# davidfang00/opticalflowdiffusion

Hardware: AMD Instinct MI355X
Metric: UNet denoise steps/sec @ 2x436x1024 flow, bs=16 (higher is better)
Workload: dtype bf16

## Files before the change

opticalflowdiffusion_amd/csrc/attn_bwd.hip:

```cpp
#include "blocks.h"

namespace ofd {

typedef __attribute__((ext_vector_type(8))) __bf16 bf16x8;
typedef __attribute__((ext_vector_type(16))) float f32x16;

__device__ __forceinline__ void a_unpack8(const uint4& v, float* f) {
    const uint32_t w[4] = {v.x, v.y, v.z, v.w};
#pragma unroll
    for (int j = 0; j < 4; ++j) {
        f[2 * j] = bf2f((bf16_t)(w[j] & 0xffffu));
        f[2 * j + 1] = bf2f((bf16_t)(w[j] >> 16));
    }
}
__device__ __forceinline__ uint4 a_pack8(const float* f) {
    return make_uint4(f2bf2(f[0], f[1]), f2bf2(f[2], f[3]), f2bf2(f[4], f[5]), f2bf2(f[6], f[7]));
}
__device__ __forceinline__ void load32(const bf16_t* p, float (&f)[32]) {
#pragma unroll
    for (int u = 0; u < 4; ++u) a_unpack8(*(const uint4*)(p + u * 8), &f[u * 8]);
}
__device__ __forceinline__ void store32(bf16_t* p, const float (&f)[32]) {
#pragma unroll
    for (int u = 0; u < 4; ++u) *(uint4*)(p + u * 8) = a_pack8(&f[u * 8]);
}

__global__ void __launch_bounds__(256) fa_bwd_delta_kernel(const bf16_t* __restrict__ o, const bf16_t* __restrict__ dout, float* __restrict__ delta, int n, size_t total) {
    for (size_t i = (size_t)blockIdx.x * 256 + threadIdx.x; i < total; i += (size_t)gridDim.x * 256) {
        const size_t pix = i >> 2;
        const int h = (int)(i & 3);
        float a[32], g[32];
        load32(o + pix * 128 + h * 32, a);
        load32(dout + pix * 128 + h * 32, g);
        float s = 0.0f;
#pragma unroll
        for (int j = 0; j < 32; ++j) s += a[j] * g[j];
        const size_t b = pix / n, q = pix % n;
        delta[(b * 4 + h) * n + q] = s;
    }
}

constexpr int FB_T = 64;
__device__ __forceinline__ int perm_slot(int idx) {
    const int kb = idx >> 5, kk = idx & 31, s = kk >> 4, a = (kk >> 3) & 1, hh = (kk >> 2) & 1, bb = kk & 3;
    return kb * 32 + s * 16 + hh * 8 + a * 4 + bb;
}
__device__ __forceinline__ void stage_transposed(unsigned char* lds, int u, int slot, const uint4& v) {
    const uint32_t w[4] = {v.x, v.y, v.z, v.w};
#pragma unroll
    for (int j = 0; j < 4; ++j) {
        *(bf16_t*)(lds + (u * 8 + 2 * j) * 144 + slot * 2) = (bf16_t)(w[j] & 0xffffu);
        *(bf16_t*)(lds + (u * 8 + 2 * j + 1) * 144 + slot * 2) = (bf16_t)(w[j] >> 16);
    }
}
__device__ __forceinline__ bf16x8 acc_to_bf16(const f32x16& a, int s) {
    bf16x8 f;
#pragma unroll
    for (int j = 0; j < 8; ++j) f[j] = (__bf16)a[8 * s + j];
    return f;
}

__global__ void __launch_bounds__(256) fa_bwd_dq_kernel(const bf16_t* __restrict__ qkv, const bf16_t* __restrict__ dout, const float* __restrict__ lse,
                                                        const float* __restrict__ delta, bf16_t* __restrict__ dqkv, int n, float scale) {
    __shared__ __attribute__((aligned(16))) unsigned char k_lds[FB_T * 80], v_lds[FB_T * 80], kt_lds[32 * 144];
    const int tid = threadIdx.x, lane = tid & 63, wave = tid >> 6, l31 = lane & 31, half = lane >> 5;
    const int bh = blockIdx.y, b = bh / 4, h = bh % 4;
    const int q0 = blockIdx.x * 128 + wave * 32;
    const bf16_t* base = qkv + (size_t)b * n * 384;
    const int qi = min(q0 + l31, n - 1);
    bf16x8 qf[2], gf[2];
#pragma unroll
    for (int s = 0; s < 2; ++s) {
        qf[s] = *(const bf16x8*)(base + (size_t)qi * 384 + h * 32 + s * 16 + half * 8);
        gf[s] = *(const bf16x8*)(dout + ((size_t)b * n + qi) * 128 + h * 32 + s * 16 + half * 8);
    }
    const float c2 = scale * 1.4426950408889634f;
    const float lse_q = lse[(size_t)bh * n + qi] * 1.4426950408889634f, dl_q = delta[(size_t)bh * n + qi] * scale;
    f32x16 dq_acc;
#pragma unroll
    for (int r = 0; r < 16; ++r) dq_acc[r] = 0.0f;
    for (int j0 = 0; j0 < n; j0 += FB_T) {
        __syncthreads();
        {
            const int key = tid >> 2, u = tid & 3;
            const int kg = min(j0 + key, n - 1);
            const uint4 kv = *(const uint4*)(base + (size_t)kg * 384 + 128 + h * 32 + u * 8);
            const uint4 vv = *(const uint4*)(base + (size_t)kg * 384 + 256 + h * 32 + u * 8);
            *(uint4*)(k_lds + key * 80 + u * 16) = kv;
            *(uint4*)(v_lds + key * 80 + u * 16) = vv;
            stage_transposed(kt_lds, u, perm_slot(key), kv);
        }
        __syncthreads();
#pragma unroll
        for (int kb = 0; kb < 2; ++kb) {
            f32x16 s_acc, p_acc;
#pragma unroll
            for (int r = 0; r < 16; ++r) { s_acc[r] = 0.0f; p_acc[r] = 0.0f; }
#pragma unroll
            for (int s = 0; s < 2; ++s) {
                const bf16x8 kf = *(const bf16x8*)(k_lds + (kb * 32 + l31) * 80 + (s * 16 + half * 8) * 2);
                const bf16x8 vf = *(const bf16x8*)(v_lds + (kb * 32 + l31) * 80 + (s * 16 + half * 8) * 2);
                s_acc = __builtin_amdgcn_mfma_f32_32x32x16_bf16(kf, qf[s], s_acc, 0, 0, 0);
                p_acc = __builtin_amdgcn_mfma_f32_32x32x16_bf16(vf, gf[s], p_acc, 0, 0, 0);
            }
#pragma unroll
            for (int r = 0; r < 16; ++r)
                s_acc[r] = __builtin_amdgcn_exp2f(__builtin_fmaf(s_acc[r], c2, -lse_q)) * __builtin_fmaf(p_acc[r], scale, -dl_q);
            if (j0 + FB_T > n) {
#pragma unroll
                for (int r = 0; r < 16; ++r)
                    if (j0 + kb * 32 + (r & 3) + 8 * (r >> 2) + 4 * half >= n) s_acc[r] = 0.0f;
            }
#pragma unroll
            for (int s = 0; s < 2; ++s) {
                const bf16x8 ktf = *(const bf16x8*)(kt_lds + l31 * 144 + (kb * 32 + s * 16 + half * 8) * 2);
                dq_acc = __builtin_amdgcn_mfma_f32_32x32x16_bf16(ktf, acc_to_bf16(s_acc, s), dq_acc, 0, 0, 0);
            }
        }
    }
    const int q = q0 + l31;
    if (q < n) {
        bf16_t* dst = dqkv + ((size_t)b * n + q) * 384 + h * 32;
#pragma unroll
        for (int g = 0; g < 4; ++g)
            *(uint2*)(dst + 8 * g + 4 * half) = make_uint2(f2bf2(dq_acc[4 * g], dq_acc[4 * g + 1]), f2bf2(dq_acc[4 * g + 2], dq_acc[4 * g + 3]));
    }
}

__global__ void __launch_bounds__(256) fa_bwd_dkv_kernel(const bf16_t* __restrict__ qkv, const bf16_t* __restrict__ dout, const float* __restrict__ lse,
                                                         const float* __restrict__ delta, bf16_t* __restrict__ dqkv, int n, float scale) {
    __shared__ __attribute__((aligned(16))) unsigned char q_lds[FB_T * 80], g_lds[FB_T * 80], qt_lds[32 * 144], gt_lds[32 * 144];
    __shared__ float lse_s[FB_T], dl_s[FB_T];
    const int tid = threadIdx.x, lane = tid & 63, wave = tid >> 6, l31 = lane & 31, half = lane >> 5;
    const int bh = blockIdx.y, b = bh / 4, h = bh % 4;
    const int k0 = blockIdx.x * 128 + wave * 32;
    const bf16_t* base = qkv + (size_t)b * n * 384;
    const int ki = min(k0 + l31, n - 1);
    bf16x8 kf[2], vf[2];
#pragma unroll
    for (int s = 0; s < 2; ++s) {
        kf[s] = *(const bf16x8*)(base + (size_t)ki * 384 + 128 + h * 32 + s * 16 + half * 8);
        vf[s] = *(const bf16x8*)(base + (size_t)ki * 384 + 256 + h * 32 + s * 16 + half * 8);
    }
    f32x16 dk_acc, dv_acc;
#pragma unroll
    for (int r = 0; r < 16; ++r) { dk_acc[r] = 0.0f; dv_acc[r] = 0.0f; }
    const float c2 = scale * 1.4426950408889634f;
    for (int i0 = 0; i0 < n; i0 += FB_T) {
        __syncthreads();
        {
            const int qq = tid >> 2, u = tid & 3;
            const bool ok = i0 + qq < n;
            const int qg = min(i0 + qq, n - 1);
            const uint4 qv = *(const uint4*)(base + (size_t)qg * 384 + h * 32 + u * 8);
            uint4 gv = *(const uint4*)(dout + ((size_t)b * n + qg) * 128 + h * 32 + u * 8);
            if (!ok) gv = make_uint4(0u, 0u, 0u, 0u);
            *(uint4*)(q_lds + qq * 80 + u * 16) = qv;
            *(uint4*)(g_lds + qq * 80 + u * 16) = gv;
            const int slot = perm_slot(qq);
            stage_transposed(qt_lds, u, slot, qv);
            stage_transposed(gt_lds, u, slot, gv);
            if (u == 0) {
                lse_s[qq] = ok ? lse[(size_t)bh * n + qg] * 1.4426950408889634f : 3.0e38f;
                dl_s[qq] = ok ? delta[(size_t)bh * n + qg] * scale : 0.0f;
            }
        }
        __syncthreads();
#pragma unroll
        for (int qb = 0; qb < 2; ++qb) {
            f32x16 s_acc, p_acc;
#pragma unroll
            for (int r = 0; r < 16; ++r) { s_acc[r] = 0.0f; p_acc[r] = 0.0f; }
#pragma unroll
            for (int s = 0; s < 2; ++s) {
                const bf16x8 qfr = *(const bf16x8*)(q_lds + (qb * 32 + l31) * 80 + (s * 16 + half * 8) * 2);
                const bf16x8 gfr = *(const bf16x8*)(g_lds + (qb * 32 + l31) * 80 + (s * 16 + half * 8) * 2);
                s_acc = __builtin_amdgcn_mfma_f32_32x32x16_bf16(qfr, kf[s], s_acc, 0, 0, 0);
                p_acc = __builtin_amdgcn_mfma_f32_32x32x16_bf16(gfr, vf[s], p_acc, 0, 0, 0);
            }
#pragma unroll
            for (int r = 0; r < 16; ++r) {
                const int qq = qb * 32 + (r & 3) + 8 * (r >> 2) + 4 * half;
                const float p = __builtin_amdgcn_exp2f(__builtin_fmaf(s_acc[r], c2, -lse_s[qq]));
                s_acc[r] = p;
                p_acc[r] = p * __builtin_fmaf(p_acc[r], scale, -dl_s[qq]);
            }
#pragma unroll
            for (int s = 0; s < 2; ++s) {
                const bf16x8 gtf = *(const bf16x8*)(gt_lds + l31 * 144 + (qb * 32 + s * 16 + half * 8) * 2);
                const bf16x8 qtf = *(const bf16x8*)(qt_lds + l31 * 144 + (qb * 32 + s * 16 + half * 8) * 2);
                dv_acc = __builtin_amdgcn_mfma_f32_32x32x16_bf16(gtf, acc_to_bf16(s_acc, s), dv_acc, 0, 0, 0);
                dk_acc = __builtin_amdgcn_mfma_f32_32x32x16_bf16(qtf, acc_to_bf16(p_acc, s), dk_acc, 0, 0, 0);
            }
        }
    }
    const int key = k0 + l31;
    if (key < n) {
        bf16_t* dst = dqkv + ((size_t)b * n + key) * 384 + h * 32;
#pragma unroll
        for (int g = 0; g < 4; ++g) {
            *(uint2*)(dst + 128 + 8 * g + 4 * half) = make_uint2(f2bf2(dk_acc[4 * g], dk_acc[4 * g + 1]), f2bf2(dk_acc[4 * g + 2], dk_acc[4 * g + 3]));
            *(uint2*)(dst + 256 + 8 * g + 4 * half) = make_uint2(f2bf2(dv_acc[4 * g], dv_acc[4 * g + 1]), f2bf2(dv_acc[4 * g + 2], dv_acc[4 * g + 3]));
        }
    }
}

int k_flash_attention_bwd(const bf16_t* qkv, const bf16_t* o, const bf16_t* dout, const float* lse, bf16_t* dqkv, float* delta, int B, int n,
                          hipStream_t s) {
    const size_t total = (size_t)B * n * 4;
    size_t gb = (total + 255) / 256;
    if (gb > 4096) gb = 4096;
    const float scale = 0.17677669529663687f;
    fa_bwd_delta_kernel<<<(int)gb, 256, 0, s>>>(o, dout, delta, n, total);
    fa_bwd_dq_kernel<<<dim3(cdiv(n, 128), B * 4), 256, 0, s>>>(qkv, dout, lse, delta, dqkv, n, scale);
    fa_bwd_dkv_kernel<<<dim3(cdiv(n, 128), B * 4), 256, 0, s>>>(qkv, dout, lse, delta, dqkv, n, scale);
    OFD_LAUNCH_CHECK();
    return OFD_OK;
}

}
using namespace ofd;

extern "C" size_t ofd_la_workspace_floats(int B, int n) { return (size_t)B * 4 * (size_t)la_fwd_parts(B, n) * 1088; }
extern "C" size_t ofd_la_bwd_workspace_floats(int B, int n) { return la_bwd_workspace_floats(B, n); }
extern "C" int ofd_linear_attention_core(const void* qkv, void* out, float* ctx, float* ml, float* workspace, int B, int n, void* stream) {
    OFD_CHECK_ARG(qkv && out && ctx && ml && workspace && B > 0 && n > 0, "linear_attention_core: bad argument");
    return k_linear_attention_core((const bf16_t*)qkv, workspace, ctx, (bf16_t*)out, B, n, (hipStream_t)stream, ml);
}
extern "C" int ofd_linear_attention_core_backward(const void* qkv, const void* dout, const float* ctx, const float* ml, void* dqkv, float* workspace,
                                                  int B, int n, void* stream) {
    OFD_CHECK_ARG(qkv && dout && ctx && ml && dqkv && workspace && B > 0 && n > 0, "linear_attention_core_backward: bad argument");
    return k_linear_attention_core_bwd((const bf16_t*)qkv, (const bf16_t*)dout, ctx, ml, (bf16_t*)dqkv, workspace, B, n, (hipStream_t)stream);
}
static inline bool al16(const void* p) { return ((uintptr_t)p & 15) == 0; }
extern "C" int ofd_la_weight_prep(const float* wqkv, const float* g, const float* wout, void* wq, void* wkv, void* woutp, int C, void* stream) {
    OFD_CHECK_ARG(wqkv && wq && wkv && (woutp == nullptr) == (wout == nullptr), "la_weight_prep: null argument (wout and woutp go together)");
    OFD_CHECK_ARG(C == 64 || C == 128, "la_weight_prep: C=%d (64 or 128)", C);
    OFD_CHECK_ARG(al16(wq) && al16(wkv) && al16(woutp), "la_weight_prep: weight buffers must be 16-byte aligned");
    return k_la_weight_prep(wqkv, g, wout, (bf16_t*)wq, (bf16_t*)wkv, (bf16_t*)woutp, C, (hipStream_t)stream);
}
extern "C" int ofd_linear_attention_block(const void* x, const void* wq, const void* wkv, const void* woutp, const float* bias, const float* g2,
                                          float* partial, void* ctxfrag, void* y, int B, int n, int C, float eps_pre, float eps_post, void* stream) {
    OFD_CHECK_ARG(x && wq && wkv && woutp && bias && g2 && partial && ctxfrag && y, "linear_attention_block: null argument");
    OFD_CHECK_ARG(C == 64 || C == 128, "linear_attention_block: C=%d (64 or 128)", C);
    OFD_CHECK_ARG(B > 0 && n > 0, "linear_attention_block: B=%d n=%d", B, n);
    OFD_CHECK_ARG(al16(x) && al16(y) && al16(wq) && al16(wkv) && al16(woutp) && al16(ctxfrag), "linear_attention_block: x, y, ctxfrag and the weights must be 16-byte aligned");
    return k_linear_attention_fused((const bf16_t*)x, (const bf16_t*)wq, (const bf16_t*)wkv, (const bf16_t*)woutp, bias, g2, partial, (bf16_t*)ctxfrag,
                                    (bf16_t*)y, B, n, C, eps_pre, eps_post, (hipStream_t)stream);
}
extern "C" int ofd_linear_attention_block_train(const void* x, const void* wq, const void* wkv, const void* woutp, const float* bias, const float* g_pre,
                                                const float* g2, float* partial, void* ctxfrag, float* ctx, float* ml, void* xn, void* qkv, void* o2,
                                                void* y, int B, int n, int C, float eps_pre, float eps_post, void* stream) {
    OFD_CHECK_ARG(x && wq && wkv && woutp && bias && g_pre && g2 && partial && ctxfrag && ctx && ml && xn && qkv && o2 && y,
                  "linear_attention_block_train: null argument");
    OFD_CHECK_ARG(C == 64, "linear_attention_block_train: C=%d (64)", C);
    OFD_CHECK_ARG(B > 0 && n > 0, "linear_attention_block_train: B=%d n=%d", B, n);
    OFD_CHECK_ARG(al16(x) && al16(y) && al16(wq) && al16(wkv) && al16(woutp) && al16(ctxfrag) && al16(xn) && al16(qkv) && al16(o2),
                  "linear_attention_block_train: x, y, xn, qkv, o2, ctxfrag and the weights must be 16-byte aligned");
    return k_linear_attention_fused_train((const bf16_t*)x, (const bf16_t*)wq, (const bf16_t*)wkv, (const bf16_t*)woutp, bias, g_pre, g2, partial,
                                          (bf16_t*)ctxfrag, ctx, ml, (bf16_t*)xn, (bf16_t*)qkv, (bf16_t*)o2, (bf16_t*)y, B, n, C, eps_pre, eps_post,
                                          (hipStream_t)stream);
}
extern "C" int ofd_linear_attention_core_proj(const void* qkv, void* out, float* ctx, float* ml, float* workspace, const void* wo, const float* bo,
                                              void* o2, int C, int B, int n, void* stream) {
    OFD_CHECK_ARG(qkv && ctx && ml && workspace && wo && o2, "linear_attention_core_proj: null argument");
    OFD_CHECK_ARG(C == 128, "linear_attention_core_proj: C=%d (128: the only width the executor runs this form at)", C);
    OFD_CHECK_ARG(B > 0 && n > 0, "linear_attention_core_proj: B=%d n=%d", B, n);
    OFD_CHECK_ARG(al16(qkv) && al16(out) && al16(wo) && al16(o2) && al16(bo), "linear_attention_core_proj: qkv, out, o2, wo and bo must be 16-byte aligned");
    return k_linear_attention_core((const bf16_t*)qkv, workspace, ctx, (bf16_t*)out, B, n, (hipStream_t)stream, ml, (const bf16_t*)wo, bo, (bf16_t*)o2, C);
}
extern "C" int ofd_linear_attention_block_backward(const void* qkv, const void* do2, const float* ctx, const float* ml, float* workspace, const void* xn,
                                                   const void* wqkv_t, float* dw_acc, void* dxn, const void* wo_fwd, const void* wo_t, float* dwo_acc,
                                                   float* dbo, const void* wq_fwd, int C, int B, int n, void* stream) {
    OFD_CHECK_ARG(qkv && do2 && ctx && ml && workspace && xn && wqkv_t && dw_acc && dxn && wo_fwd && wo_t && dwo_acc && dbo && wq_fwd,
                  "linear_attention_block_backward: null argument");
    OFD_CHECK_ARG(C == 64, "linear_attention_block_backward: C=%d (64)", C);
    OFD_CHECK_ARG(B > 0 && n > 0, "linear_attention_block_backward: B=%d n=%d", B, n);
    OFD_CHECK_ARG(al16(qkv) && al16(do2) && al16(xn) && al16(dxn) && al16(wqkv_t) && al16(wo_fwd) && al16(wo_t) && al16(wq_fwd),
                  "linear_attention_block_backward: qkv, do2, xn, dxn and the weights must be 16-byte aligned");
    return k_linear_attention_block_bwd((const bf16_t*)qkv, (const bf16_t*)do2, ctx, ml, workspace, B, n, (hipStream_t)stream, (const bf16_t*)xn,
                                        (const bf16_t*)wqkv_t, dw_acc, (bf16_t*)dxn, (const bf16_t*)wo_fwd, (const bf16_t*)wo_t, dwo_acc, dbo,
                                        (const bf16_t*)wq_fwd);
}
extern "C" int ofd_flash_attention(const void* qkv, void* out, float* lse, int B, int n, void* stream) {
    OFD_CHECK_ARG(qkv && out && B > 0 && n > 0, "flash_attention: bad argument");
    return k_flash_attention((const bf16_t*)qkv, (bf16_t*)out, B, n, (hipStream_t)stream, lse);
}
extern "C" int ofd_flash_attention_backward(const void* qkv, const void* out, const void* dout, const float* lse, void* dqkv, float* delta, int B,
                                            int n, void* stream) {
    OFD_CHECK_ARG(qkv && out && dout && lse && dqkv && delta && B > 0 && n > 0, "flash_attention_backward: bad argument");
    return k_flash_attention_bwd((const bf16_t*)qkv, (const bf16_t*)out, (const bf16_t*)dout, lse, (bf16_t*)dqkv, delta, B, n, (hipStream_t)stream);
}
```

opticalflowdiffusion_amd/csrc/blocks.h:

```cpp
#pragma once
#include "common.h"

namespace ofd {

struct MlpDesc {
    const float* weight;
    const float* bias;
    int n_out;
    int offset;
};

struct FcFuse { const float* w; const float* b; float* out; };
bool conv_fc_fuse_supported(const ofd_conv_args* a, int out_dim);
int conv_forward_impl(const ofd_conv_args* a, hipStream_t s, int pool2 = 0, const bf16_t* residual_b = nullptr, const FcFuse* fc = nullptr);
bool conv_pool2_supported(const ofd_conv_args* a);
bool conv_residual_b_supported(const ofd_conv_args* a);
int k_wt_transpose(const bf16_t* w, bf16_t* wt, int taps, int Cin, int Cout, hipStream_t s);
int k_conv_wgrad(const ofd_conv_args* a, const bf16_t* dy, float* dw, hipStream_t s, float* dbias = nullptr);
int k_conv7_wgrad(const bf16_t* x16, const bf16_t* dy, float* dw, int B, int H, int W, hipStream_t s, float* dbias = nullptr, int channels = 16);
int k_channel_sum(const bf16_t* dy, float* out, size_t npix, int C, hipStream_t s);
int k_wgrad_finish(const float* acc, const float* w_raw, float* dst, int Cout, int Cin, int Cin_pad, int ksize, float ws_eps, int unshuffle,
                   int accumulate, hipStream_t s);
int k_grad_scatter(const bf16_t* D, int Ctot, int ch_off, bf16_t* dst, int C, int B, int H, int W, int mode, int p1, int p2, int accumulate,
                   hipStream_t s);

struct ofd_weight_prep_desc {
    const float* w;
    void* out;
    int Cout, Cin, Cin_pad, ksize;
    float ws_eps;
    int unshuffle;
    int block0;
};
int k_conv_weight_prep_batched(const ofd_weight_prep_desc* d_descs, int n, int total_blocks, hipStream_t s);
int k_wt_transpose_batched(const ofd_weight_prep_desc* d_descs, int n, int total_blocks, hipStream_t s);
int k_pack_input(const float* x, int Cx, const float* cond, int Cc, bf16_t* out, int B, int H, int W, hipStream_t s, int cpad = 16, int ax = 0, int ac = 0);
int k_time_mlp(const int64_t* t, const float* w1, const float* b1, const float* w2, const float* b2, float* temb,
               float* temb_silu, int B, int dim, hipStream_t s);
int k_block_mlp(const float* temb_silu, const MlpDesc* descs, int n_desc, float* ss, int B, int tdim, int ss_stride, hipStream_t s);
int k_gn_finalize(const float* partial, int B, int H, int W, int C, const float* gamma, const float* beta, const float* ss,
                  int ss_stride, int ss_offset, float* a_out, float* s_out, hipStream_t s, float* stats_out = nullptr);
int k_resblock_out(const bf16_t* h, const float* a, const float* sft, const bf16_t* x, bf16_t* out, int B, int H, int W, int C, hipStream_t s);
int k_layernorm_c(const bf16_t* x, const float* g, const bf16_t* res, bf16_t* out, size_t npix, int C, float eps, hipStream_t s);
int la_parts(int B, int n);
int k_linear_attention_core(const bf16_t* qkv, float* partial, float* ctx, bf16_t* out, int B, int n, hipStream_t s, float* ml_out = nullptr,
                            const bf16_t* wo = nullptr, const float* bo = nullptr, bf16_t* o2 = nullptr, int C = 0);
int la_fused_blocks(int n, int B);
int la_fwd_parts(int B, int n);
int k_linear_attention_fused_train(const bf16_t* x, const bf16_t* wq, const bf16_t* wkv, const bf16_t* woutp, const float* bias, const float* g_pre,
                                   const float* g2, float* partial, bf16_t* ctxfrag, float* ctx, float* ml, bf16_t* xn, bf16_t* qkv, bf16_t* o2,
                                   bf16_t* y, int B, int n, int C, float eps_pre, float eps_post, hipStream_t s);
int k_la_weight_prep(const float* wqkv, const float* g, const float* wout, bf16_t* wq, bf16_t* wkv, bf16_t* woutp, int C, hipStream_t s);
int k_linear_attention_fused(const bf16_t* x, const bf16_t* wq, const bf16_t* wkv, const bf16_t* woutp, const float* bias, const float* g2,
                             float* partial, bf16_t* ctxfrag, bf16_t* y, int B, int n, int C, float eps_pre, float eps_post, hipStream_t s);
int k_flash_attention(const bf16_t* qkv, bf16_t* out, int B, int n, hipStream_t s, float* lse = nullptr);
int k_final_conv(const bf16_t* x, const float* w, const float* bias, float* out, int B, int H, int W, int C, int out_dim, hipStream_t s, int out_mode = 0,
                 float out_div = 1.0f);
int k_nhwc_to_nchw(const bf16_t* x, float* out, int B, int H, int W, int C, hipStream_t s);
int k_nchw_to_nhwc(const float* x, bf16_t* out, int B, int H, int W, int C, hipStream_t s);

int k_affine_silu(const bf16_t* h, const float* a, const float* s, bf16_t* out, int B, int H, int W, int C, hipStream_t st);
size_t gn_bwd_workspace_floats(int B, int H, int W, int C);
int k_gn_silu_backward(const bf16_t* g, const bf16_t* h, const float* a, const float* s, const float* stats, const float* gamma,
                       const float* beta, const float* ss, int ss_stride, int ss_offset, bf16_t* dh, float* dgamma, float* dbeta, float* dss,
                       float* workspace, int B, int H, int W, int C, hipStream_t st, float* dconv_bias = nullptr);
int k_layernorm_c_bwd(const bf16_t* x, const float* gw, const bf16_t* dy, bf16_t* dx, float* dg, size_t npix, int C, float eps, int accumulate,
                      hipStream_t st, const bf16_t* extra = nullptr);
int k_final_conv_bwd(const bf16_t* x, const float* w, const float* dy, bf16_t* dx, float* dw, float* db, int B, int H, int W, int C, int out_dim,
                     hipStream_t st, const float* bias = nullptr, int out_mode = 0, float out_div = 1.0f);
int k_conv7_dgrad(const bf16_t* dy, const bf16_t* wt, int cin_pad, float* dx, int cx, int B, int H, int W, float scale, hipStream_t s);
int k_block_mlp_bwd(const float* dss, const float* temb_silu, const float* weight, int n_out, int offset, float* dweight, float* dbias, float* dts,
                    int B, int tdim, int ss_stride, hipStream_t st);
int k_time_mlp_bwd(const int64_t* t, const float* temb, const float* dts, const float* w1, const float* b1, const float* w2, float* dw1, float* db1,
                   float* dw2, float* db2, float* scratch, int B, int dim, hipStream_t st);
int k_grad_add(bf16_t* dst, const bf16_t* src, size_t elems, int accumulate, hipStream_t st);

size_t la_bwd_workspace_floats(int B, int n);
int k_linear_attention_core_bwd(const bf16_t* qkv, const bf16_t* dout, const float* ctx, const float* ml, bf16_t* dqkv, float* workspace, int B, int n,
                                hipStream_t s);
int k_linear_attention_block_bwd(const bf16_t* qkv, const bf16_t* do2, const float* ctx, const float* ml, float* workspace, int B, int n, hipStream_t s,
                                 const bf16_t* xn, const bf16_t* wt, float* dw, bf16_t* dxn, const bf16_t* wo_fwd, const bf16_t* wo_t, float* dwo,
                                 float* dbo, const bf16_t* wq);
int k_flash_attention_bwd(const bf16_t* qkv, const bf16_t* o, const bf16_t* dout, const float* lse, bf16_t* dqkv, float* delta, int B, int n,
                          hipStream_t s);

}
```

opticalflowdiffusion_amd/csrc/la_fused.hip:

```cpp
#include <cstdlib>
#include <type_traits>
#include "blocks.h"
#include "la_common.h"

namespace ofd {

template <int C>
struct XRaw {
    u32x4 v[C / 16];
};

template <int C>
__device__ __forceinline__ void load_raw_x(const bf16_t* __restrict__ xrow, XRaw<C>& r, int half) {
#pragma unroll
    for (int s = 0; s < C / 16; ++s) r.v[s] = *(const u32x4*)(xrow + 16 * s + 8 * half);
}

typedef __bf16 la_bf16x2 __attribute__((ext_vector_type(2)));
template <int C>
__device__ __forceinline__ void norm_stats(const XRaw<C>& r, float eps, float& rstd, float& off) {
    const la_bf16x2 one = __builtin_bit_cast(la_bf16x2, 0x3f803f80u);
    float s1 = 0.0f, s2 = 0.0f;
#pragma unroll
    for (int s = 0; s < C / 16; ++s)
#pragma unroll
        for (int j = 0; j < 4; ++j) {
            const la_bf16x2 w = __builtin_bit_cast(la_bf16x2, (uint32_t)r.v[s][j]);
            s1 = __builtin_amdgcn_fdot2_f32_bf16(w, one, s1, false);
            s2 = __builtin_amdgcn_fdot2_f32_bf16(w, w, s2, false);
        }
    s1 += __shfl_xor(s1, 32, 64);
    s2 += __shfl_xor(s2, 32, 64);
    const float mean = s1 * (1.0f / C);
    const float var = fmaxf(__builtin_fmaf(-mean, mean, s2 * (1.0f / C)), 0.0f);
    rstd = rsqrtf(var + eps);
    off = -mean * rstd;
}
template <int C>
__device__ __forceinline__ void norm_x(const XRaw<C>& r, float eps, bf16x8 (&xs)[C / 16]) {
    float rstd, off;
    norm_stats<C>(r, eps, rstd, off);
#pragma unroll
    for (int s = 0; s < C / 16; ++s)
#pragma unroll
        for (int j = 0; j < 4; ++j) {
            const uint32_t w = r.v[s][j];
            xs[s][2 * j] = (__bf16)__builtin_fmaf(bf2f((bf16_t)(w & 0xffffu)), rstd, off);
            xs[s][2 * j + 1] = (__bf16)__builtin_fmaf(bf2f((bf16_t)(w >> 16)), rstd, off);
        }
}

template <int C>
__device__ __forceinline__ void norm_x_gain(const XRaw<C>& r, float eps, const float* __restrict__ g, int half, bf16x8 (&xs)[C / 16]) {
    float rstd, off;
    norm_stats<C>(r, eps, rstd, off);
#pragma unroll
    for (int s = 0; s < C / 16; ++s) {
        const float4 g0 = *(const float4*)(g + 16 * s + 8 * half), g1 = *(const float4*)(g + 16 * s + 8 * half + 4);
        const float gg[8] = {g0.x, g0.y, g0.z, g0.w, g1.x, g1.y, g1.z, g1.w};
#pragma unroll
        for (int j = 0; j < 4; ++j) {
            const uint32_t w = r.v[s][j];
            xs[s][2 * j] = (__bf16)(__builtin_fmaf(bf2f((bf16_t)(w & 0xffffu)), rstd, off) * gg[2 * j]);
            xs[s][2 * j + 1] = (__bf16)(__builtin_fmaf(bf2f((bf16_t)(w >> 16)), rstd, off) * gg[2 * j + 1]);
        }
    }
}

constexpr int LA_PART_PITCH = 64 + 32 * 36;
__device__ __forceinline__ void la_store_part(float* lds, float* __restrict__ o, float m, float l, const f32x16& ctxT, int tid, int wave, int l31,
                                              int half) {
    float* mine = lds + wave * LA_PART_PITCH;
    const float l_tot = l + __shfl_xor(l, 32, 64);
    if (half == 0) {
        mine[l31] = m;
        mine[32 + l31] = l_tot;
    }
#pragma unroll
    for (int g = 0; g < 4; ++g)
        *(float4*)(mine + 64 + l31 * 36 + 8 * g + 4 * half) = make_float4(ctxT[4 * g], ctxT[4 * g + 1], ctxT[4 * g + 2], ctxT[4 * g + 3]);
    __syncthreads();
    const int d = tid >> 3, e0 = (tid & 7) * 4;
    float mw[4], M = -3.0e38f;
#pragma unroll
    for (int w = 0; w < 4; ++w) {
        mw[w] = lds[w * LA_PART_PITCH + d];
        M = fmaxf(M, mw[w]);
    }
    float4 a = make_float4(0.0f, 0.0f, 0.0f, 0.0f);
    float ls = 0.0f;
#pragma unroll
    for (int w = 0; w < 4; ++w) {
        const float wt = __expf(mw[w] - M);
        const float4 v = *(const float4*)(lds + w * LA_PART_PITCH + 64 + d * 36 + e0);
        a.x += v.x * wt;
        a.y += v.y * wt;
        a.z += v.z * wt;
        a.w += v.w * wt;
        ls += lds[w * LA_PART_PITCH + 32 + d] * wt;
    }
    *(float4*)(o + 64 + d * 32 + e0) = a;
    if ((tid & 7) == 0) {
        o[d] = M;
        o[32 + d] = ls;
    }
    __syncthreads();
}

__device__ __forceinline__ void ctx_state_init(f32x16 (&ctxT)[4], float (&m)[4], float (&l)[4]) {
#pragma unroll
    for (int hd = 0; hd < 4; ++hd) {
        m[hd] = -3.0e38f;
        l[hd] = 0.0f;
#pragma unroll
        for (int r = 0; r < 16; ++r) ctxT[hd][r] = 0.0f;
    }
}
__device__ __forceinline__ f32x16 ctx_mask_rows(f32x16 ka, int tile, int n, int half) {
    if (tile * 32 + 32 > n) {
#pragma unroll
        for (int r = 0; r < 16; ++r)
            if (tile * 32 + acc_row(r, half) >= n) ka[r] = -3.0e38f;
    }
    return ka;
}
__device__ __forceinline__ float ctx_tile_max(const f32x16& ka) {
    float mt = -3.0e38f;
#pragma unroll
    for (int r = 0; r < 16; ++r) mt = fmaxf(mt, ka[r]);
    return fmaxf(mt, __shfl_xor(mt, 32, 64));
}
__device__ __forceinline__ void ctx_update(f32x16& ctxT, const f32x16& va, const f32x16& p) {
#pragma unroll
    for (int s2 = 0; s2 < 2; ++s2) ctxT = __builtin_amdgcn_mfma_f32_32x32x16_bf16(acc_frag(va, s2), acc_frag(p, s2), ctxT, 0, 0, 0);
}

template <int C, bool TRAIN>
__global__ void __launch_bounds__(256, 2) la_ctx_fused_kernel(const bf16_t* __restrict__ x, const bf16_t* __restrict__ wkv,
                                                           float* __restrict__ partial, int n, float eps, float defer,
                                                           const float* __restrict__ g, bf16_t* __restrict__ xn_out, bf16_t* __restrict__ qkv_out) {
    extern __shared__ __attribute__((aligned(16))) unsigned char smem[];
    constexpr int KS = C / 16;
    const int tid = threadIdx.x, lane = tid & 63, wave = tid >> 6, l31 = lane & 31, half = lane >> 5;
    for (int i = tid; i < (C / 8) * 256; i += 256) ((uint4*)smem)[i] = ((const uint4*)wkv)[i];
    float* s_g = (float*)(smem + (C / 8) * 256 * 16);
    if constexpr (TRAIN)
        for (int i = tid; i < C; i += 256) s_g[i] = g[i];
    __syncthreads();
    const int b = blockIdx.y, wave_id = blockIdx.x * 4 + wave, nw = gridDim.x * 4, ntiles = (n + 31) / 32;

    f32x16 ctxT[4];
    float m[4], l[4];
    ctx_state_init(ctxT, m, l);
    const bf16_t* xb = x + (size_t)b * n * C;
    XRaw<C> raw_next;
    load_raw_x<C>(xb + (size_t)min(wave_id * 32 + l31, n - 1) * C, raw_next, half);
    for (int tile = wave_id; tile < ntiles; tile += nw) {
        asm volatile("" ::: "memory");
        const XRaw<C> raw = raw_next;
        load_raw_x<C>(xb + (size_t)min((tile + nw) * 32 + l31, n - 1) * C, raw_next, half);
        bf16x8 xs[KS];
        const int pix = tile * 32 + l31;
        if constexpr (TRAIN) {
            norm_x_gain<C>(raw, eps, s_g, half, xs);
            if (pix < n) {
                bf16_t* xrow = xn_out + ((size_t)b * n + pix) * C;
#pragma unroll
                for (int s = 0; s < KS; ++s) *(bf16x8*)(xrow + 16 * s + 8 * half) = xs[s];
            }
        } else {
            norm_x<C>(raw, eps, xs);
        }
        if constexpr (TRAIN) {
            bf16_t* qrow = qkv_out + ((size_t)b * n + min(pix, n - 1)) * 384 + 128;
#pragma unroll
            for (int blk = 0; blk < 8; ++blk) {
                f32x16 t;
#pragma unroll
                for (int r = 0; r < 16; ++r) t[r] = 0.0f;
#pragma unroll
                for (int s = 0; s < KS; ++s)
                    t = __builtin_amdgcn_mfma_f32_32x32x16_bf16(*(const bf16x8*)(smem + ((size_t)(2 * s + half) * 256 + blk * 32 + l31) * 16), xs[s], t, 0, 0, 0);
                store_acc_rows(t, qrow + blk * 32, half, pix < n);
            }
        }
#pragma unroll
        for (int hd = 0; hd < 4; ++hd) {
            f32x16 ka, va;
#pragma unroll
            for (int r = 0; r < 16; ++r) { ka[r] = 0.0f; va[r] = 0.0f; }
#pragma unroll
            for (int s = 0; s < KS; ++s) {
                const bf16x8 wk = *(const bf16x8*)(smem + ((size_t)(2 * s + half) * 256 + hd * 32 + l31) * 16);
                const bf16x8 wv = *(const bf16x8*)(smem + ((size_t)(2 * s + half) * 256 + 128 + hd * 32 + l31) * 16);
                ka = __builtin_amdgcn_mfma_f32_32x32x16_bf16(xs[s], wk, ka, 0, 0, 0);
                va = __builtin_amdgcn_mfma_f32_32x32x16_bf16(xs[s], wv, va, 0, 0, 0);
            }
            if constexpr (TRAIN) {
#pragma unroll
                for (int r = 0; r < 16; ++r) ka[r] = bf2f(f2bf(ka[r]));
            }
            ka = ctx_mask_rows(ka, tile, n, half);
            const float mt = ctx_tile_max(ka);
            const bool move = mt > m[hd] + defer;
            if (__builtin_amdgcn_ballot_w64(move)) {
                const float m_new = move ? mt : m[hd];
                const float f = __expf(m[hd] - m_new);
                m[hd] = m_new;
                l[hd] *= f;
#pragma unroll
                for (int r = 0; r < 16; ++r) ctxT[hd][r] *= f;
            }
            float ps = 0.0f;
            const float m2 = m[hd] * LA_LOG2E;
#pragma unroll
            for (int r = 0; r < 16; ++r) {
                const float p = __builtin_amdgcn_exp2f(__builtin_fmaf(ka[r], LA_LOG2E, -m2));
                ka[r] = p;
                ps += p;
            }
            l[hd] += ps;
            ctx_update(ctxT[hd], va, ka);
            if constexpr (TRAIN) {
#pragma unroll
                for (int r = 0; r < 16; ++r) ka[r] -= (float)(__bf16)ka[r];
                ctx_update(ctxT[hd], va, ka);
            }
        }
    }
    __syncthreads();
#pragma unroll
    for (int hd = 0; hd < 4; ++hd)
        la_store_part((float*)smem, partial + ((size_t)(b * 4 + hd) * gridDim.x + blockIdx.x) * 1088, m[hd], l[hd], ctxT[hd], tid, wave, l31, half);
}

__global__ void __launch_bounds__(256, 2) la_ctx_stored_kernel(const bf16_t* __restrict__ qkv, float* __restrict__ partial, int n) {
    const int tid = threadIdx.x, lane = tid & 63, wave = tid >> 6, l31 = lane & 31, half = lane >> 5;
    const int b = blockIdx.y, wave_id = blockIdx.x * 4 + wave, nw = gridDim.x * 4, ntiles = (n + 31) / 32;
    bf16x8 ident[2];
#pragma unroll
    for (int s2 = 0; s2 < 2; ++s2)
#pragma unroll
        for (int j = 0; j < 8; ++j) ident[s2][j] = (__bf16)((16 * s2 + 8 * half + j == l31) ? 1.0f : 0.0f);
    f32x16 ctxT[4];
    float m[4], l[4];
    ctx_state_init(ctxT, m, l);
    const bf16_t* qb = qkv + (size_t)b * n * 384;
    for (int tile = wave_id; tile < ntiles; tile += nw) {
        u32x4 kr[8], vr[8];
        {
            const bf16_t* row = qb + (size_t)min(tile * 32 + l31, n - 1) * 384 + 128 + 8 * half;
#pragma unroll
            for (int i = 0; i < 8; ++i) kr[i] = *(const u32x4*)(row + 16 * i);
#pragma unroll
            for (int i = 0; i < 8; ++i) vr[i] = *(const u32x4*)(row + 128 + 16 * i);
        }
#pragma unroll
        for (int hd = 0; hd < 4; ++hd) {
            f32x16 ka, va;
#pragma unroll
            for (int r = 0; r < 16; ++r) { ka[r] = 0.0f; va[r] = 0.0f; }
#pragma unroll
            for (int s2 = 0; s2 < 2; ++s2) {
                ka = __builtin_amdgcn_mfma_f32_32x32x16_bf16(__builtin_bit_cast(bf16x8, kr[hd * 2 + s2]), ident[s2], ka, 0, 0, 0);
                va = __builtin_amdgcn_mfma_f32_32x32x16_bf16(__builtin_bit_cast(bf16x8, vr[hd * 2 + s2]), ident[s2], va, 0, 0, 0);
            }
            ka = ctx_mask_rows(ka, tile, n, half);
            const float mt = ctx_tile_max(ka);
            const float m_new = fmaxf(m[hd], mt);
            const float f = __expf(m[hd] - m_new);
            m[hd] = m_new;
            float ps = 0.0f;
            const float m2 = m_new * LA_LOG2E;
#pragma unroll
            for (int r = 0; r < 16; ++r) {
                const float p = bf2f(f2bf(__builtin_amdgcn_exp2f(__builtin_fmaf(ka[r], LA_LOG2E, -m2))));
                ka[r] = p;
                ps += p;
            }
            l[hd] = l[hd] * f + ps;
#pragma unroll
            for (int r = 0; r < 16; ++r) ctxT[hd][r] *= f;
            ctx_update(ctxT[hd], va, ka);
        }
    }
    __shared__ __attribute__((aligned(16))) float part_s[4 * LA_PART_PITCH];
#pragma unroll
    for (int hd = 0; hd < 4; ++hd)
        la_store_part(part_s, partial + ((size_t)(b * 4 + hd) * gridDim.x + blockIdx.x) * 1088, m[hd], l[hd], ctxT[hd], tid, wave, l31, half);
}

int launch_la_ctx_stored(const bf16_t* qkv, float* partial, int B, int n, hipStream_t s) {
    const int gx = la_fused_blocks(n, B);
    la_ctx_stored_kernel<<<dim3(gx, B), 256, 0, s>>>(qkv, partial, n);
    return gx;
}

constexpr int LA_MAX_PARTS = 256;
template <class Out>
__global__ void __launch_bounds__(256) la_ctx_combine_kernel(const float* __restrict__ partial, Out* __restrict__ out, int nparts, float inv_n,
                                                             float* __restrict__ ml_out) {
    constexpr bool FRAG = std::is_same<Out, bf16_t>::value;
    __shared__ float red[8][32], M[32], Linv[32], w_s[LA_MAX_PARTS][32];
    const int tid = threadIdx.x, bh = blockIdx.x, dd = tid & 31, grp = tid >> 5;
    const float* base = partial + (size_t)bh * nparts * 1088;
    float mx = -3.0e38f;
    for (int c0 = grp; c0 < nparts; c0 += 32) {
        float t[4];
#pragma unroll
        for (int k = 0; k < 4; ++k) t[k] = base[(size_t)min(c0 + 8 * k, nparts - 1) * 1088 + dd];
#pragma unroll
        for (int k = 0; k < 4; ++k) mx = fmaxf(mx, t[k]);
    }
    red[grp][dd] = mx;
    __syncthreads();
    if (tid < 32) {
        float m = red[0][tid];
#pragma unroll
        for (int g = 1; g < 8; ++g) m = fmaxf(m, red[g][tid]);
        M[tid] = m;
    }
    __syncthreads();
    const bool use_ws = nparts <= LA_MAX_PARTS;
    float l = 0.0f;
    for (int c0 = grp; c0 < nparts; c0 += 32) {
        float tm[4], tl[4];
#pragma unroll
        for (int k = 0; k < 4; ++k) {
            const size_t o = (size_t)min(c0 + 8 * k, nparts - 1) * 1088;
            tm[k] = base[o + dd];
            tl[k] = base[o + 32 + dd];
        }
#pragma unroll
        for (int k = 0; k < 4; ++k)
            if (c0 + 8 * k < nparts) {
                const float w = __expf(tm[k] - M[dd]);
                if (use_ws) w_s[c0 + 8 * k][dd] = w;
                l += tl[k] * w;
            }
    }
    __syncthreads();
    red[grp][dd] = l;
    __syncthreads();
    if (tid < 32) {
        float t = red[0][tid];
#pragma unroll
        for (int g = 1; g < 8; ++g) t += red[g][tid];
        Linv[tid] = 1.0f / t;
        if (!FRAG && ml_out && blockIdx.y == 0) {
            ml_out[(size_t)bh * 64 + tid] = M[tid];
            ml_out[(size_t)bh * 64 + 32 + tid] = 1.0f / t;
        }
    }
    __syncthreads();
    const int i = blockIdx.y * 256 + tid;
    int d, e;
    if constexpr (FRAG) {
        const int j = i & 7, lane = (i >> 3) & 63, s2 = i >> 9;
        d = 16 * s2 + 8 * (j >> 2) + 4 * (lane >> 5) + (j & 3);
        e = lane & 31;
    } else {
        d = i >> 5;
        e = i & 31;
    }
    float a = 0.0f;
    for (int c0 = 0; c0 < nparts; c0 += 8) {
        float v[8];
#pragma unroll
        for (int k = 0; k < 8; ++k) v[k] = base[(size_t)min(c0 + k, nparts - 1) * 1088 + 64 + d * 32 + e];
        if (use_ws) {
#pragma unroll
            for (int k = 0; k < 8; ++k)
                if (c0 + k < nparts) a += v[k] * w_s[c0 + k][d];
        } else {
            float mc[8];
#pragma unroll
            for (int k = 0; k < 8; ++k) mc[k] = base[(size_t)min(c0 + k, nparts - 1) * 1088 + d];
#pragma unroll
            for (int k = 0; k < 8; ++k)
                if (c0 + k < nparts) a += v[k] * __expf(mc[k] - M[d]);
        }
    }
    const float c = a * Linv[d] * inv_n;
    if constexpr (FRAG) out[(size_t)bh * 1024 + i] = f2bf(c);
    else out[(size_t)bh * 1024 + i] = c;
}
void launch_la_ctx_combine(const float* partial, float* ctx, int B, int nparts, float inv_n, float* ml_out, hipStream_t s) {
    la_ctx_combine_kernel<<<dim3(B * 4, 4), 256, 0, s>>>(partial, ctx, nparts, inv_n, ml_out);
}

template <int C, bool TRAIN>
__global__ void __launch_bounds__(256, C == 64 ? 4 : 2) la_out_fused_kernel(const bf16_t* __restrict__ x, const bf16_t* __restrict__ wq,
                                                           const bf16_t* __restrict__ woutp, const bf16_t* __restrict__ ctxfrag,
                                                           const float* __restrict__ bias, const float* __restrict__ g2,
                                                           bf16_t* __restrict__ y, int n, float eps_pre, float eps_post, float scale,
                                                           const float* __restrict__ g, bf16_t* __restrict__ o2_out) {
    extern __shared__ __attribute__((aligned(16))) unsigned char smem[];
    constexpr int KS = C / 16, RT = C / 32;
    constexpr int WQ_B = (C / 8) * 128 * 16, WO_B = 16 * C * 16, CF_B = 4 * 2 * 64 * 16;
    unsigned char* s_wq = smem;
    unsigned char* s_wo = smem + WQ_B;
    unsigned char* s_cf = s_wo + WO_B;
    float* s_bias = (float*)(s_cf + CF_B);
    float* s_g2 = s_bias + C;
    float* s_g = s_g2 + C;
    const int tid = threadIdx.x, lane = tid & 63, wave = tid >> 6, l31 = lane & 31, half = lane >> 5;
    const int b = blockIdx.y;
    if constexpr (TRAIN)
        for (int i = tid; i < C; i += 256) s_g[i] = g[i];
    for (int i = tid; i < WQ_B / 16; i += 256) ((uint4*)s_wq)[i] = ((const uint4*)wq)[i];
    for (int i = tid; i < WO_B / 16; i += 256) ((uint4*)s_wo)[i] = ((const uint4*)woutp)[i];
    for (int i = tid; i < CF_B / 16; i += 256) ((uint4*)s_cf)[i] = ((const uint4*)(ctxfrag + (size_t)b * 4096))[i];
    for (int i = tid; i < C; i += 256) { s_bias[i] = bias[i]; s_g2[i] = g2[i]; }
    __syncthreads();
    const int wave_id = blockIdx.x * 4 + wave, nw = gridDim.x * 4, ntiles = (n + 31) / 32;

    const bf16_t* xb = x + (size_t)b * n * C;
    XRaw<C> raw_next;
    load_raw_x<C>(xb + (size_t)min(wave_id * 32 + l31, n - 1) * C, raw_next, half);
    for (int tile = wave_id; tile < ntiles; tile += nw) {
        asm volatile("" ::: "memory");
        const int pix = tile * 32 + l31;
        const int pid = min(pix, n - 1);
        const bf16_t* xrow = xb + (size_t)pid * C;
        const XRaw<C> raw = raw_next;
        load_raw_x<C>(xb + (size_t)min((tile + nw) * 32 + l31, n - 1) * C, raw_next, half);
        bf16x8 xs[KS];
        if constexpr (TRAIN) norm_x_gain<C>(raw, eps_pre, s_g, half, xs);
        else norm_x<C>(raw, eps_pre, xs);
        f32x16 acc_o[RT];
#pragma unroll
        for (int rt = 0; rt < RT; ++rt)
#pragma unroll
            for (int r = 0; r < 16; ++r) acc_o[rt][r] = 0.0f;
#pragma unroll
        for (int hd = 0; hd < 4; ++hd) {
            f32x16 qa;
#pragma unroll
            for (int r = 0; r < 16; ++r) qa[r] = 0.0f;
#pragma unroll
            for (int s = 0; s < KS; ++s) {
                const bf16x8 wf = *(const bf16x8*)(s_wq + ((size_t)(2 * s + half) * 128 + hd * 32 + l31) * 16);
                qa = __builtin_amdgcn_mfma_f32_32x32x16_bf16(wf, xs[s], qa, 0, 0, 0);
            }
            if constexpr (TRAIN) {
#pragma unroll
                for (int r = 0; r < 16; ++r) qa[r] = bf2f(f2bf(qa[r]));
            }
            const float k = scale / softmax_d(qa, 32);
#pragma unroll
            for (int r = 0; r < 16; ++r) qa[r] *= k;
            f32x16 oa;
#pragma unroll
            for (int r = 0; r < 16; ++r) oa[r] = 0.0f;
#pragma unroll
            for (int s2 = 0; s2 < 2; ++s2) {
                const bf16x8 cf = *(const bf16x8*)(s_cf + ((size_t)(hd * 2 + s2) * 64 + lane) * 16);
                oa = __builtin_amdgcn_mfma_f32_32x32x16_bf16(cf, acc_frag(qa, s2), oa, 0, 0, 0);
            }
#pragma unroll
            for (int s2 = 0; s2 < 2; ++s2) {
                const bf16x8 of = acc_frag(oa, s2);
#pragma unroll
                for (int rt = 0; rt < RT; ++rt) {
                    const bf16x8 wf = *(const bf16x8*)(s_wo + ((size_t)((hd * 2 + s2) * 2 + half) * C + rt * 32 + l31) * 16);
                    acc_o[rt] = __builtin_amdgcn_mfma_f32_32x32x16_bf16(wf, of, acc_o[rt], 0, 0, 0);
                }
            }
        }
        float sum = 0.0f;
#pragma unroll
        for (int rt = 0; rt < RT; ++rt)
#pragma unroll
            for (int g = 0; g < 4; ++g) {
                const float4 bv = *(const float4*)(s_bias + rt * 32 + 8 * g + 4 * half);
                acc_o[rt][4 * g] += bv.x; acc_o[rt][4 * g + 1] += bv.y; acc_o[rt][4 * g + 2] += bv.z; acc_o[rt][4 * g + 3] += bv.w;
                if constexpr (TRAIN) {
#pragma unroll
                    for (int k = 0; k < 4; ++k) acc_o[rt][4 * g + k] = bf2f(f2bf(acc_o[rt][4 * g + k]));
                }
                sum += (acc_o[rt][4 * g] + acc_o[rt][4 * g + 1]) + (acc_o[rt][4 * g + 2] + acc_o[rt][4 * g + 3]);
            }
        if constexpr (TRAIN) {
            bf16_t* orow = o2_out + ((size_t)b * n + min(pix, n - 1)) * C;
#pragma unroll
            for (int rt = 0; rt < RT; ++rt) store_acc_rows(acc_o[rt], orow + rt * 32, half, pix < n);
        }
        sum += __shfl_xor(sum, 32, 64);
        const float mean = sum * (1.0f / C);
        float q = 0.0f;
#pragma unroll
        for (int rt = 0; rt < RT; ++rt)
#pragma unroll
            for (int r = 0; r < 16; ++r) { acc_o[rt][r] -= mean; q += acc_o[rt][r] * acc_o[rt][r]; }
        q += __shfl_xor(q, 32, 64);
        const float rstd = rsqrtf(q * (1.0f / C) + eps_post);
        {
            const bool ok = pix < n;
            bf16_t* yrow = y + ((size_t)b * n + min(pix, n - 1)) * C;
#pragma unroll
            for (int rt = 0; rt < RT; ++rt)
#pragma unroll
                for (int g = 0; g < 4; g += 2) {
                    const u32x4 xw = raw.v[rt * 2 + (g >> 1)];
                    const uint4 xv = make_uint4(xw[0], xw[1], xw[2], xw[3]);
                    const auto sx = __builtin_amdgcn_permlane32_swap(xv.x, xv.z, false, false);
                    const auto sy = __builtin_amdgcn_permlane32_swap(xv.y, xv.w, false, false);
                    const unsigned xq[2][2] = {{sx[0], sy[0]}, {sx[1], sy[1]}};
                    uint2 qo[2];
#pragma unroll
                    for (int k = 0; k < 2; ++k) {
                        const int c0 = rt * 32 + 8 * (g + k) + 4 * half;
                        const float4 gv = *(const float4*)(s_g2 + c0);
                        const float o0 = acc_o[rt][4 * (g + k)] * rstd * gv.x + bf2f((bf16_t)(xq[k][0] & 0xffffu));
                        const float o1 = acc_o[rt][4 * (g + k) + 1] * rstd * gv.y + bf2f((bf16_t)(xq[k][0] >> 16));
                        const float o2 = acc_o[rt][4 * (g + k) + 2] * rstd * gv.z + bf2f((bf16_t)(xq[k][1] & 0xffffu));
                        const float o3 = acc_o[rt][4 * (g + k) + 3] * rstd * gv.w + bf2f((bf16_t)(xq[k][1] >> 16));
                        qo[k] = pack_quad(o0, o1, o2, o3);
                    }
                    store_quad_pair(yrow + rt * 32 + 8 * g, qo[0], qo[1], half, ok);
                }
        }
    }
}

__global__ void __launch_bounds__(256) la_weight_prep_kernel(const float* __restrict__ wqkv, const float* __restrict__ g, const float* __restrict__ wout,
                                                             bf16_t* __restrict__ wq, bf16_t* __restrict__ wkv, bf16_t* __restrict__ woutp, int C) {
    const int total = 512 * C;
    for (int i = blockIdx.x * blockDim.x + threadIdx.x; i < total; i += gridDim.x * blockDim.x) {
        if (i < 128 * C) {
            const int j = i & 7, o = (i >> 3) & 127, c8 = i >> 10, c = c8 * 8 + j;
            wq[i] = f2bf(wqkv[(size_t)o * C + c] * (g ? g[c] : 1.0f));
        } else if (i < 384 * C) {
            const int k = i - 128 * C;
            const int j = k & 7, o = (k >> 3) & 255, c8 = k >> 11, c = c8 * 8 + j;
            wkv[k] = f2bf(wqkv[(size_t)(128 + o) * C + c] * (g ? g[c] : 1.0f));
        } else if (woutp) {
            const int k = i - 384 * C;
            const int j = k & 7, c = (k >> 3) % C, rest = (k >> 3) / C;
            const int hh = rest & 1, s2 = (rest >> 1) & 1, hd = rest >> 2;
            woutp[k] = f2bf(wout[(size_t)c * 128 + hd * 32 + 16 * s2 + 8 * (j >> 2) + 4 * hh + (j & 3)]);
        }
    }
}

constexpr float LA_DEFER = 5.545177f;
constexpr int LA_GX2_CAP = 128;
static int la_out_blocks(int n, int B) {
    int gx2 = cdiv(cdiv(n, 32), 4 * 4);
    if (gx2 < 1) gx2 = 1;
    const int cap2 = (LA_GX2_CAP * B < 1024) ? 1024 / B : LA_GX2_CAP;
    if (gx2 > cap2) gx2 = cap2;
    return gx2;
}

template <int C>
static int launch_la(const bf16_t* x, const bf16_t* wq, const bf16_t* wkv, const bf16_t* woutp, const float* bias, const float* g2,
                     float* partial, bf16_t* ctxfrag, bf16_t* y, int B, int n, float eps_pre, float eps_post, hipStream_t s) {
    constexpr int LDS1 = (C / 8) * 256 * 16;
    constexpr int LDS2 = (C / 8) * 128 * 16 + 16 * C * 16 + 4 * 2 * 64 * 16 + 2 * C * 4;
    static bool attr = false;
    if (!attr) {
        OFD_HIP(hipFuncSetAttribute((const void*)la_ctx_fused_kernel<C, false>, hipFuncAttributeMaxDynamicSharedMemorySize, LDS1));
        OFD_HIP(hipFuncSetAttribute((const void*)la_out_fused_kernel<C, false>, hipFuncAttributeMaxDynamicSharedMemorySize, LDS2));
        attr = true;
    }
    const int gx = la_fused_blocks(n, B);
    la_ctx_fused_kernel<C, false><<<dim3(gx, B), 256, LDS1, s>>>(x, wkv, partial, n, eps_pre, LA_DEFER, nullptr, nullptr, nullptr);
    la_ctx_combine_kernel<<<dim3(B * 4, 4), 256, 0, s>>>(partial, ctxfrag, gx, 1.0f / (float)n, nullptr);
    la_out_fused_kernel<C, false><<<dim3(la_out_blocks(n, B), B), 256, LDS2, s>>>(x, wq, woutp, ctxfrag, bias, g2, y, n, eps_pre, eps_post, LA_SCALE, nullptr, nullptr);
    OFD_LAUNCH_CHECK();
    return OFD_OK;
}

int k_linear_attention_fused_train(const bf16_t* x, const bf16_t* wq, const bf16_t* wkv, const bf16_t* woutp, const float* bias, const float* g_pre,
                                   const float* g2, float* partial, bf16_t* ctxfrag, float* ctx, float* ml, bf16_t* xn, bf16_t* qkv, bf16_t* o2,
                                   bf16_t* y, int B, int n, int C, float eps_pre, float eps_post, hipStream_t s) {
    if (C != 64) { set_error("linear_attention_fused_train: C=%d unsupported", C); return OFD_ERR_ARG; }
    constexpr int LDS1 = (64 / 8) * 256 * 16 + 64 * 4;
    constexpr int LDS2 = (64 / 8) * 128 * 16 + 16 * 64 * 16 + 4 * 2 * 64 * 16 + 3 * 64 * 4;
    static bool attr = false;
    if (!attr) {
        OFD_HIP(hipFuncSetAttribute((const void*)la_ctx_fused_kernel<64, true>, hipFuncAttributeMaxDynamicSharedMemorySize, LDS1));
        OFD_HIP(hipFuncSetAttribute((const void*)la_out_fused_kernel<64, true>, hipFuncAttributeMaxDynamicSharedMemorySize, LDS2));
        attr = true;
    }
    const int gx = la_fused_blocks(n, B);
    la_ctx_fused_kernel<64, true><<<dim3(gx, B), 256, LDS1, s>>>(x, wkv, partial, n, eps_pre, LA_DEFER, g_pre, xn, qkv);
    la_ctx_combine_kernel<<<dim3(B * 4, 4), 256, 0, s>>>(partial, ctxfrag, gx, 1.0f / (float)n, nullptr);
    launch_la_ctx_combine(partial, ctx, B, gx, 1.0f / (float)n, ml, s);
    la_out_fused_kernel<64, true><<<dim3(la_out_blocks(n, B), B), 256, LDS2, s>>>(x, wq, woutp, ctxfrag, bias, g2, y, n, eps_pre, eps_post, LA_SCALE, g_pre, o2);
    OFD_LAUNCH_CHECK();
    return OFD_OK;
}

int la_fused_blocks(int n, int B) {
    constexpr int total = 256;
    int gx = cdiv(cdiv(n, 32), 8);
    int cap = total / (B < 1 ? 1 : B);
    if (cap < 64) cap = 64;
    if (gx < 1) gx = 1;
    if (gx > cap) gx = cap;
    return gx;
}

int k_la_weight_prep(const float* wqkv, const float* g, const float* wout, bf16_t* wq, bf16_t* wkv, bf16_t* woutp, int C, hipStream_t s) {
    la_weight_prep_kernel<<<cdiv((woutp ? 512 : 384) * C, 256), 256, 0, s>>>(wqkv, g, wout, wq, wkv, woutp, C);
    OFD_LAUNCH_CHECK();
    return OFD_OK;
}

int k_linear_attention_fused(const bf16_t* x, const bf16_t* wq, const bf16_t* wkv, const bf16_t* woutp, const float* bias, const float* g2,
                             float* partial, bf16_t* ctxfrag, bf16_t* y, int B, int n, int C, float eps_pre, float eps_post, hipStream_t s) {
    if (C == 64) return launch_la<64>(x, wq, wkv, woutp, bias, g2, partial, ctxfrag, y, B, n, eps_pre, eps_post, s);
    if (C == 128) return launch_la<128>(x, wq, wkv, woutp, bias, g2, partial, ctxfrag, y, B, n, eps_pre, eps_post, s);
    set_error("linear_attention_fused: C=%d unsupported", C);
    return OFD_ERR_ARG;
}

}
```

opticalflowdiffusion_amd/csrc/unet.hip:

```cpp
#include <cstdlib>
#include "unet_exec.h"

using namespace ofd;

namespace ofd {

float site_eps(const ofd_unet* u, const std::string& site) {
    if (u->cfg.eps_mode == 0) return 1e-5f;
    auto ends = [&](const char* s) { std::string t(s); return site.size() >= t.size() && site.compare(site.size() - t.size(), t.size(), t) == 0; };
    if (ends(".fn.fn.to_out.1")) return 1e-3f;
    if (ends(".0.block1.proj") && site.rfind("downs.", 0) == 0) return 1e-3f;
    if (site == "mid_block1.block1.proj" || site == "final_res_block.block1.proj") return 1e-3f;
    return 1e-5f;
}

static void add_param(ofd_unet* u, const std::string& name, std::vector<int> shape) {
    size_t numel = 1;
    for (int d : shape) numel *= (size_t)d;
    Param p{name, (int)shape.size(), {1, 1, 1, 1}, numel, u->n_param_floats, false};
    for (size_t i = 0; i < shape.size(); ++i) p.shape[i] = shape[i];
    u->pindex[name] = (int)u->params.size();
    u->params.push_back(p);
    u->n_param_floats += (numel + 3) / 4 * 4;
}

static void add_conv(ofd_unet* u, const std::string& prefix, int co, int ci, int k, bool bias, float ws_eps, int unshuffle = 0) {
    add_param(u, prefix + ".weight", {co, ci, k, k});
    if (bias) add_param(u, prefix + ".bias", {co});
    ConvDesc c{prefix + ".weight", co, ci, (k == 7) ? (ci + 15) / 16 * 16 : ci, k, ws_eps, unshuffle, u->n_wbuf};
    u->n_wbuf += (size_t)k * k * c.Cin_pad * co;
    if (k == 7 && ci <= 8) {
        c.pack8_off = (long)u->n_wbuf;
        u->n_wbuf += ofd_conv_weight_elems(co, 8, 7);
    }
    u->cindex[prefix] = (int)u->convs.size();
    u->convs.push_back(c);
}

static void add_resblock(ofd_unet* u, const std::string& name, int ci, int co) {
    const int tdim = u->cfg.dim * 4;
    if (!u->cfg.no_time) {
        add_param(u, name + ".mlp.1.weight", {co * 2, tdim});
        add_param(u, name + ".mlp.1.bias", {co * 2});
    }
    add_conv(u, name + ".block1.proj", co, ci, 3, true, site_eps(u, name + ".block1.proj"));
    add_param(u, name + ".block1.norm.weight", {co});
    add_param(u, name + ".block1.norm.bias", {co});
    add_conv(u, name + ".block2.proj", co, co, 3, true, site_eps(u, name + ".block2.proj"));
    add_param(u, name + ".block2.norm.weight", {co});
    add_param(u, name + ".block2.norm.bias", {co});
    if (ci != co) add_conv(u, name + ".res_conv", co, ci, 1, true, -1.0f);
    u->ss_offset[name] = u->ss_stride;
    u->ss_stride += 2 * co;
}

static void add_linattn(ofd_unet* u, const std::string& name, int c) {
    add_conv(u, name + ".fn.fn.to_qkv", 384, c, 1, false, -1.0f);
    add_conv(u, name + ".fn.fn.to_out.0", c, 128, 1, true, -1.0f);
    add_param(u, name + ".fn.fn.to_out.1.g", {1, c, 1, 1});
    add_param(u, name + ".fn.norm.g", {1, c, 1, 1});
    if (c <= 128) {
        u->la_fused[name] = {u->n_labuf, c};
        u->n_labuf += (size_t)512 * c;
        if (c == 64) u->n_labuf += (size_t)384 * c;
    }
}

static void build_registry(ofd_unet* u) {
    const int dim = u->cfg.dim, L = u->L;
    u->dims = {dim, dim, dim * 2, dim * 4};
    if (L == 4) u->dims.push_back(dim * 8);
    const int tdim = dim * 4;
    add_conv(u, "init_conv", dim, u->cfg.channels, 7, true, -1.0f);
    u->cin_pad = u->convs.back().Cin_pad;
    if (!u->cfg.no_time) {
        add_param(u, "time_mlp.1.weight", {tdim, dim});
        add_param(u, "time_mlp.1.bias", {tdim});
        add_param(u, "time_mlp.3.weight", {tdim, tdim});
        add_param(u, "time_mlp.3.bias", {tdim});
    }
    for (int i = 0; i < L; ++i) {
        const int ci = u->dims[i], co = u->dims[i + 1];
        const std::string p = "downs." + std::to_string(i);
        add_resblock(u, p + ".0", ci, ci);
        add_resblock(u, p + ".1", ci, ci);
        add_linattn(u, p + ".2", ci);
        if (i < L - 1) add_conv(u, p + ".3.1", co, ci * 4, 1, true, -1.0f, 1);
        else add_conv(u, p + ".3", co, ci, 3, true, -1.0f);
    }
    for (int i = 0; i < L; ++i) {
        const int ci = u->dims[L - 1 - i], co = u->dims[L - i];
        const std::string p = "ups." + std::to_string(i);
        add_resblock(u, p + ".0", co + ci, co);
        add_resblock(u, p + ".1", co + ci, co);
        add_linattn(u, p + ".2", co);
        if (i < L - 1) {
            add_conv(u, p + ".3.1", ci, co, 3, true, -1.0f);
            ConvDesc& d = u->convs.back();
            d.phase_off = (long)u->n_wbuf;
            u->n_wbuf += (size_t)16 * co * ci;
        }
        else add_conv(u, p + ".3", ci, co, 3, true, -1.0f);
    }
    const int mid = u->dims[L];
    add_resblock(u, "mid_block1", mid, mid);
    add_conv(u, "mid_attn.fn.fn.to_qkv", 384, mid, 1, false, -1.0f);
    add_conv(u, "mid_attn.fn.fn.to_out", mid, 128, 1, true, -1.0f);
    add_param(u, "mid_attn.fn.norm.g", {1, mid, 1, 1});
    add_resblock(u, "mid_block2", mid, mid);
    add_resblock(u, "final_res_block", dim * 2, dim);
    add_param(u, "final_conv.weight", {u->cfg.out_dim, dim, 1, 1});
    add_param(u, "final_conv.bias", {u->cfg.out_dim});
    for (auto& kv : u->ss_offset) u->resblocks.push_back(kv.first);
}

void conv(Ctx& c, const std::string& prefix, const std::vector<SrcSpec>& srcs, Tensor out, const float* in_scale,
                 const float* in_shift, const bf16_t* residual, const bf16_t* res_act, const float* res_scale,
                 const float* res_shift, float* gn_partial, const FcFuse* fc) {
    if (c.rc != OFD_OK) return;
    const ConvDesc& d = c.u->convs[c.u->cindex.at(prefix)];
    ofd_conv_args a{};
    a.B = c.B; a.H = out.H; a.W = out.W; a.ksize = d.ksize; a.n_src = (int)srcs.size(); a.Cout = d.Cout;
    int cin = 0;
    for (size_t i = 0; i < srcs.size(); ++i) {
        a.src[i].src = srcs[i].t.p;
        a.src[i].channels = srcs[i].t.C;
        a.src[i].src_channels = srcs[i].t.C;
        a.src[i].ch_offset = 0;
        a.src[i].upsample = srcs[i].upsample;
        a.src[i].unshuffle = srcs[i].unshuffle;
        a.src[i].p1 = srcs[i].p1;
        a.src[i].p2 = srcs[i].p2;
        cin += srcs[i].t.C;
    }
    const bool pack8 = d.ksize == 7 && cin == 8 && d.pack8_off >= 0;
    if (cin != d.Cin_pad && !pack8) { set_error("conv %s: got %d input channels, expected %d", prefix.c_str(), cin, d.Cin_pad); c.rc = OFD_ERR_ARG; return; }
    a.weight = c.u->d_wbuf + (pack8 ? (size_t)d.pack8_off : d.w_off);
    a.bias = c.u->P(prefix + ".bias");
    a.in_scale = in_scale; a.in_shift = in_shift; a.residual = residual; a.res_act = res_act;
    a.res_scale = res_scale; a.res_shift = res_shift; a.out = out.p; a.gn_partial = gn_partial;
    const double px = (double)c.B * out.H * out.W;
    const double flops = 2.0 * px * d.Cout * (double)d.Cin * d.ksize * d.ksize;
    const double bytes = px * 2.0 * (d.Cout + (double)cin / ((srcs[0].upsample) ? 4 : 1)) + (double)d.ksize * d.ksize * d.Cin_pad * d.Cout * 2.0;
    const bool pp = d.ksize == 3 && d.Cout == 64 && cin == 64 && srcs.size() == 1 && !srcs[0].upsample && !residual && !res_act;
    const int cls3 = pp ? PC_CONV3_PP : (d.Cout % 128 == 0 ? PC_CONV3 : PC_CONV3_64);
    c.begin(d.ksize == 3 ? cls3 : (d.ksize == 1 ? PC_CONV1 : PC_CONV7), flops, bytes,
            prefix + " " + std::to_string(d.Cin) + "->" + std::to_string(d.Cout) + " @" + std::to_string(out.H) + "x" + std::to_string(out.W));
    RUN(conv_forward_impl(&a, c.s, 0, nullptr, fc));
    c.end();
}

static Tensor resblock(Ctx& c, const std::string& name, const std::vector<Tensor>& in, int Cout, bool keep_out = true, const FcFuse* fc = nullptr) {
    ofd_unet* u = c.u;
    const int H = in[0].H, W = in[0].W, B = c.B;
    std::vector<SrcSpec> srcs;
    int cin = 0;
    for (auto& t : in) { SrcSpec s; s.t = t; srcs.push_back(s); cin += t.C; }
    Tensor h1 = c.tmp(Cout, H, W), h2 = c.tmp(Cout, H, W);
    const size_t np = ofd_conv_gn_partial_count(B, H, W, Cout);
    float* p1 = c.tmpf(np);
    float* p2 = c.tmpf(np);
    float* a1 = c.train ? c.keepf((size_t)B * Cout) : c.tmpf((size_t)B * Cout);
    float* s1 = c.train ? c.keepf((size_t)B * Cout) : c.tmpf((size_t)B * Cout);
    float* a2 = c.train ? c.keepf((size_t)B * Cout) : c.tmpf((size_t)B * Cout);
    float* s2 = c.train ? c.keepf((size_t)B * Cout) : c.tmpf((size_t)B * Cout);
    float* st1 = c.train ? c.keepf((size_t)B * 16) : nullptr;
    float* st2 = c.train ? c.keepf((size_t)B * 16) : nullptr;
    Tensor out = keep_out ? c.keep(Cout, H, W) : c.tmp(Cout, H, W);
    if (c.rc != OFD_OK) return out;
    conv(c, name + ".block1.proj", srcs, h1, nullptr, nullptr, nullptr, nullptr, nullptr, nullptr, p1);
    c.begin(PC_GN, 0, (double)np * 4);
    RUN(k_gn_finalize(p1, B, H, W, Cout, u->P(name + ".block1.norm.weight"), u->P(name + ".block1.norm.bias"), c.ss, u->ss_stride,
                      u->ss_offset.at(name), a1, s1, c.s, st1));
    c.end();
    SrcSpec hs; hs.t = h1;
    constexpr int act1_min = 256;
    constexpr int act1_train_min = 128;
    const int amin = c.train ? act1_train_min : act1_min;
    Tensor act1;
    if (Cout >= amin) {
        act1 = c.tmp(Cout, H, W);
        if (c.rc != OFD_OK) return out;
        c.begin(PC_MISC, 0, (double)B * H * W * Cout * 4.0);
        RUN(k_affine_silu(h1.p, a1, s1, act1.p, B, H, W, Cout, c.s));
        c.end();
        hs.t = act1;
        conv(c, name + ".block2.proj", {hs}, h2, nullptr, nullptr, nullptr, nullptr, nullptr, nullptr, p2);
    } else
    conv(c, name + ".block2.proj", {hs}, h2, a1, s1, nullptr, nullptr, nullptr, nullptr, p2);
    c.begin(PC_GN, 0, (double)np * 4);
    RUN(k_gn_finalize(p2, B, H, W, Cout, u->P(name + ".block2.norm.weight"), u->P(name + ".block2.norm.bias"), nullptr, 0, 0, a2, s2, c.s, st2));
    c.end();
    if (cin != Cout) {
        conv(c, name + ".res_conv", srcs, out, nullptr, nullptr, nullptr, h2.p, a2, s2, nullptr, fc);
    } else {
        c.begin(PC_RESOUT, 0, (double)B * H * W * Cout * 6.0);
        RUN(k_resblock_out(h2.p, a2, s2, in[0].p, out.p, B, H, W, Cout, c.s));
        c.end();
    }
    if (c.train) {
        TapeRec r;
        r.kind = TK_RES; r.name = name; r.srcs = srcs; r.out = out; r.h1 = h1; r.h2 = h2;
        r.a1 = a1; r.s1 = s1; r.a2 = a2; r.s2 = s2; r.st1 = st1; r.st2 = st2; r.act1 = act1;
        u->tape.push_back(r);
    }
    return out;
}

static Tensor linattn(Ctx& c, const std::string& name, Tensor x) {
    ofd_unet* u = c.u;
    const int H = x.H, W = x.W, B = c.B, C = x.C, n = H * W;
    const size_t npix = (size_t)B * n;
    auto fit = u->la_fused.find(name);
    if (fit != u->la_fused.end() && !c.train) {
        const int nparts = la_fused_blocks(n, B);
        float* partial = c.tmpf((size_t)B * 4 * nparts * 1088);
        bf16_t* ctxfrag = (bf16_t*)c.tmpf((size_t)B * 2048);
        Tensor y = c.keep(C, H, W);
        if (c.rc != OFD_OK) return y;
        const bf16_t* base = u->d_labuf + fit->second.first;
        c.begin(PC_LINATTN, npix * 2.0 * (C * 384.0 + 2 * 4 * 32 * 32 + 128.0 * C), (double)npix * C * 2 * 3,
                name + " fused C=" + std::to_string(C) + " @" + std::to_string(H) + "x" + std::to_string(W));
        RUN(k_linear_attention_fused(x.p, base, base + (size_t)128 * C, base + (size_t)384 * C, u->P(name + ".fn.fn.to_out.0.bias"),
                                     u->P(name + ".fn.fn.to_out.1.g"), partial, ctxfrag, y.p, B, n, C, site_eps(u, name + ".fn.norm"),
                                     site_eps(u, name + ".fn.fn.to_out.1"), c.s));
        c.end();
        return y;
    }
    Tensor xn = c.tmp(C, H, W), qkv = c.tmp(384, H, W), ao = c.tmp(128, H, W), o2 = c.tmp(C, H, W);
    const int nparts = la_fwd_parts(B, n);
    if (c.train && fit != u->la_fused.end() && la_train_fused(C)) {
        float* partial = c.tmpf((size_t)B * 4 * nparts * 1088);
        bf16_t* ctxfrag = (bf16_t*)c.tmpf((size_t)B * 2048);
        float* ctx = c.keepf((size_t)B * 4 * 1024);
        float* ml = c.keepf((size_t)B * 4 * 64);
        Tensor y = c.keep(C, H, W);
        if (c.rc != OFD_OK) return y;
        const bf16_t* base = u->d_labuf + fit->second.first;
        c.begin(PC_LINATTN, npix * 2.0 * (C * 640.0 + 2 * 4 * 32 * 32 + 128.0 * C), (double)npix * C * 2 * (2 + 1 + 4 + 2),
                name + " fused (training) C=" + std::to_string(C) + " @" + std::to_string(H) + "x" + std::to_string(W));
        RUN(k_linear_attention_fused_train(x.p, base + (size_t)512 * C, base + (size_t)640 * C, base + (size_t)384 * C, u->P(name + ".fn.fn.to_out.0.bias"),
                                           u->P(name + ".fn.norm.g"), u->P(name + ".fn.fn.to_out.1.g"), partial, ctxfrag, ctx, ml, xn.p, qkv.p, o2.p, y.p,
                                           B, n, C, site_eps(u, name + ".fn.norm"), site_eps(u, name + ".fn.fn.to_out.1"), c.s));
        c.end();
        TapeRec r;
        r.kind = TK_LINATTN; r.name = name; r.x = x; r.xn = xn; r.qkv = qkv; r.ao = ao; r.o2 = o2; r.out = y; r.ctx = ctx; r.ml = ml;
        u->tape.push_back(r);
        return y;
    }
    float* partial = c.tmpf((size_t)B * 4 * nparts * 1088);
    float* ctx = c.train ? c.keepf((size_t)B * 4 * 1024) : c.tmpf((size_t)B * 4 * 1024);
    float* ml = c.train ? c.keepf((size_t)B * 4 * 64) : nullptr;
    Tensor y = c.keep(C, H, W);
    if (c.rc != OFD_OK) return y;
    c.begin(PC_LN, 0, (double)npix * C * 4);
    RUN(k_layernorm_c(x.p, u->P(name + ".fn.norm.g"), nullptr, xn.p, npix, C, site_eps(u, name + ".fn.norm"), c.s));
    c.end();
    SrcSpec s; s.t = xn;
    conv(c, name + ".fn.fn.to_qkv", {s}, qkv, nullptr, nullptr, nullptr, nullptr, nullptr, nullptr, nullptr);
    c.begin(PC_LINATTN, 4.0 * npix * 4 * 32 * 32, (double)npix * (384 + 128 + 128) * 2);
    if (C == 128) {
        const ConvDesc& d = u->convs[u->cindex.at(name + ".fn.fn.to_out.0")];
        RUN(k_linear_attention_core(qkv.p, partial, ctx, ao.p, B, n, c.s, ml, u->d_wbuf + d.w_off, u->P(name + ".fn.fn.to_out.0.bias"), o2.p, C));
        c.end();
    } else {
        RUN(k_linear_attention_core(qkv.p, partial, ctx, ao.p, B, n, c.s, ml));
        c.end();
        SrcSpec s2; s2.t = ao;
        conv(c, name + ".fn.fn.to_out.0", {s2}, o2, nullptr, nullptr, nullptr, nullptr, nullptr, nullptr, nullptr);
    }
    c.begin(PC_LN, 0, (double)npix * C * 6);
    RUN(k_layernorm_c(o2.p, u->P(name + ".fn.fn.to_out.1.g"), x.p, y.p, npix, C, site_eps(u, name + ".fn.fn.to_out.1"), c.s));
    c.end();
    if (c.train) {
        TapeRec r;
        r.kind = TK_LINATTN; r.name = name; r.x = x; r.xn = xn; r.qkv = qkv; r.ao = ao; r.o2 = o2; r.out = y; r.ctx = ctx; r.ml = ml;
        u->tape.push_back(r);
    }
    return y;
}

static Tensor midattn(Ctx& c, Tensor x) {
    ofd_unet* u = c.u;
    const int H = x.H, W = x.W, B = c.B, C = x.C, n = H * W;
    Tensor xn = c.tmp(C, H, W), qkv = c.tmp(384, H, W), ao = c.tmp(128, H, W);
    float* lse = c.train ? c.keepf((size_t)B * 4 * n) : nullptr;
    Tensor y = c.keep(C, H, W);
    if (c.rc != OFD_OK) return y;
    const size_t npix = (size_t)B * n;
    c.begin(PC_LN, 0, (double)npix * C * 4);
    RUN(k_layernorm_c(x.p, u->P("mid_attn.fn.norm.g"), nullptr, xn.p, npix, C, site_eps(u, "mid_attn.fn.norm"), c.s));
    c.end();
    SrcSpec s; s.t = xn;
    conv(c, "mid_attn.fn.fn.to_qkv", {s}, qkv, nullptr, nullptr, nullptr, nullptr, nullptr, nullptr, nullptr);
    c.begin(PC_FLASH, 4.0 * B * 4.0 * (double)n * n * 32, (double)npix * (384 + 128) * 2);
    RUN(k_flash_attention(qkv.p, ao.p, B, n, c.s, lse));
    c.end();
    SrcSpec s2; s2.t = ao;
    conv(c, "mid_attn.fn.fn.to_out", {s2}, y, nullptr, nullptr, x.p, nullptr, nullptr, nullptr, nullptr);
    if (c.train) {
        TapeRec r;
        r.kind = TK_MIDATTN; r.name = "mid_attn"; r.x = x; r.xn = xn; r.qkv = qkv; r.ao = ao; r.out = y; r.lse = lse;
        u->tape.push_back(r);
    }
    return y;
}

static void plain_conv(Ctx& c, const std::string& prefix, const std::vector<SrcSpec>& srcs, Tensor out) {
    conv(c, prefix, srcs, out, nullptr, nullptr, nullptr, nullptr, nullptr, nullptr, nullptr);
    if (c.train) {
        TapeRec r;
        r.kind = TK_CONV; r.name = prefix; r.srcs = srcs; r.out = out;
        c.u->tape.push_back(r);
    }
}

static void upsample_conv(Ctx& c, const std::string& prefix, const SrcSpec& src_up, Tensor out) {
    ofd_unet* u = c.u;
    const ConvDesc& d = u->convs[u->cindex.at(prefix)];
    if (d.phase_off < 0) { plain_conv(c, prefix, {src_up}, out); return; }
    if (c.rc != OFD_OK) return;
    const Tensor& lo = src_up.t;
    const double px = (double)c.B * out.H * out.W;
    c.begin(PC_CONVUP, 2.0 * px * d.Cout * (double)d.Cin * 9 , px * 2.0 * (d.Cout + d.Cin / 4.0),
            prefix + " " + std::to_string(d.Cin) + "->" + std::to_string(d.Cout) + " @" + std::to_string(out.H) + "x" + std::to_string(out.W) + " (4 phases)");
    {
        ofd_conv_args a{};
        a.B = c.B; a.H = lo.H; a.W = lo.W; a.ksize = 2; a.n_src = 1; a.Cout = d.Cout;
        a.src[0].src = lo.p; a.src[0].channels = lo.C; a.src[0].src_channels = lo.C;
        a.weight = u->d_wbuf + d.phase_off;
        a.bias = u->P(prefix + ".bias");
        a.out = out.p;
        a.up2_phase = 5;
        RUN(conv_forward_impl(&a, c.s));
    }
    c.end();
    if (c.train) {
        TapeRec r;
        r.kind = TK_CONV; r.name = prefix; r.srcs = {src_up}; r.out = out;
        u->tape.push_back(r);
    }
}

int run_forward(Ctx& c, const float* x, int Cx, const float* cond, int Cc, const int64_t* t, float* out, int H, int W, float* temb,
                float* temb_silu) {
    ofd_unet* u = c.u;
    const int B = c.B, dim = u->cfg.dim;
    u->taps.clear();
    u->last_B = B;
    if (c.train) u->tape.clear();
    const bool pack8 = u->convs[u->cindex.at("init_conv")].pack8_off >= 0;
    const int cpad = pack8 ? 8 : u->cin_pad;
    const int L = u->L;
    Tensor xin = c.keep(cpad, H, W);
    c.begin(PC_MISC, 0, 0);
    RUN(k_pack_input(x, Cx, cond, cond ? Cc : 0, xin.p, B, H, W, c.s, cpad, u->glue_x, u->glue_cond));
    if (!u->cfg.no_time) {
        RUN(k_time_mlp(t, u->P("time_mlp.1.weight"), u->P("time_mlp.1.bias"), u->P("time_mlp.3.weight"), u->P("time_mlp.3.bias"), temb, temb_silu, B, dim, c.s));
        RUN(k_block_mlp(temb_silu, u->d_mlp, (int)u->resblocks.size(), c.ss, B, dim * 4, u->ss_stride, c.s));
    } else {
        c.ss = nullptr;
    }
    c.end();
    Tensor r = c.keep(dim, H, W);
    { SrcSpec s; s.t = xin; plain_conv(c, "init_conv", {s}, r); }
    u->taps["init_conv"] = r;

    Tensor xcur = r;
    std::vector<Tensor> hs;
    for (int i = 0; i < L; ++i) {
        const std::string p = "downs." + std::to_string(i);
        c.reset_scratch();
        xcur = resblock(c, p + ".0", {xcur}, u->dims[i]);
        hs.push_back(xcur);
        u->taps[p + ".0"] = xcur;
        c.reset_scratch();
        Tensor x1 = resblock(c, p + ".1", {xcur}, u->dims[i]);
        u->taps[p + ".1"] = x1;
        c.reset_scratch();
        xcur = linattn(c, p + ".2", x1);
        hs.push_back(xcur);
        u->taps[p + ".2"] = xcur;
        if (i < L - 1) {
            Tensor d = c.keep(u->dims[i + 1], xcur.H / 2, xcur.W / 2);
            std::vector<SrcSpec> srcs;
            for (int sub = 0; sub < 4; ++sub) { SrcSpec s; s.t = xcur; s.unshuffle = 1; s.p1 = sub >> 1; s.p2 = sub & 1; srcs.push_back(s); }
            plain_conv(c, p + ".3.1", srcs, d);
            xcur = d;
        } else {
            Tensor d = c.keep(u->dims[i + 1], xcur.H, xcur.W);
            SrcSpec s; s.t = xcur;
            plain_conv(c, p + ".3", {s}, d);
            xcur = d;
        }
        u->taps[p + ".3"] = xcur;
    }
    c.reset_scratch();
    xcur = resblock(c, "mid_block1", {xcur}, u->dims[L]);
    u->taps["mid_block1"] = xcur;
    c.reset_scratch();
    xcur = midattn(c, xcur);
    u->taps["mid_attn"] = xcur;
    c.reset_scratch();
    xcur = resblock(c, "mid_block2", {xcur}, u->dims[L]);
    u->taps["mid_block2"] = xcur;
    for (int i = 0; i < L; ++i) {
        const std::string p = "ups." + std::to_string(i);
        const int co = u->dims[L - i], ci = u->dims[L - 1 - i];
        c.reset_scratch();
        Tensor h = hs.back(); hs.pop_back();
        xcur = resblock(c, p + ".0", {xcur, h}, co);
        u->taps[p + ".0"] = xcur;
        c.reset_scratch();
        h = hs.back(); hs.pop_back();
        xcur = resblock(c, p + ".1", {xcur, h}, co);
        u->taps[p + ".1"] = xcur;
        c.reset_scratch();
        xcur = linattn(c, p + ".2", xcur);
        u->taps[p + ".2"] = xcur;
        if (i < L - 1) {
            Tensor d = c.keep(ci, xcur.H * 2, xcur.W * 2);
            SrcSpec s; s.t = xcur; s.upsample = 1;
            upsample_conv(c, p + ".3.1", s, d);
            xcur = d;
        } else {
            Tensor d = c.keep(ci, xcur.H, xcur.W);
            SrcSpec s; s.t = xcur;
            plain_conv(c, p + ".3", {s}, d);
            xcur = d;
        }
        u->taps[p + ".3"] = xcur;
    }
    c.reset_scratch();
    const int glue = u->glue_out;
    const bool fuse_fc = !c.train && !u->debug_taps && !glue && u->cfg.out_dim == 2 && dim == 64 && ((long)H * W) % 128 == 0;
    if (fuse_fc) {
        const FcFuse fc{u->P("final_conv.weight"), u->P("final_conv.bias"), out};
        if (c.rc == OFD_OK && !c.dry) {
            if (hipMemsetAsync(out, 0, (size_t)B * 2 * H * W * sizeof(float), c.s) != hipSuccess) { set_error("unet_forward: hipMemsetAsync failed"); c.rc = OFD_ERR_HIP; }
            c.chain_ok = false;
        }
        xcur = resblock(c, "final_res_block", {xcur, r}, dim, true, &fc);
    } else {
        xcur = resblock(c, "final_res_block", {xcur, r}, dim);
        u->taps["final_res_block"] = xcur;
        c.begin(PC_MISC, 2.0 * B * H * W * dim * u->cfg.out_dim, (double)B * H * W * (dim * 2 + u->cfg.out_dim * 4));
        RUN(k_final_conv(xcur.p, u->P("final_conv.weight"), u->P("final_conv.bias"), out, B, H, W, dim, u->cfg.out_dim, c.s, glue, u->glue_div));
        c.end();
    }
    if (c.train) {
        u->ts.B = B; u->ts.H = H; u->ts.W = W; u->ts.t = t; u->ts.ss = c.ss; u->ts.temb = temb; u->ts.temb_silu = temb_silu;
        u->ts.xin = xin; u->ts.r = r; u->ts.xf = xcur; u->ts.persist_used = c.persist_used;
    }
    return c.rc;
}

size_t persist_bytes(const ofd_unet* u, int B, int H, int W) {
    auto T = [&](int C, int h, int w) { return ((size_t)B * h * w * C * 2 + 255) / 256 * 256; };
    const int L = u->L;
    size_t n = T(u->cin_pad, H, W) + T(u->dims[0], H, W);
    int h = H, w = W;
    for (int i = 0; i < L; ++i) {
        n += 3 * T(u->dims[i], h, w);
        if (i < L - 1) { h /= 2; w /= 2; }
        n += T(u->dims[i + 1], h, w);
    }
    n += 3 * T(u->dims[L], h, w);
    for (int i = 0; i < L; ++i) {
        const int co = u->dims[L - i], ci = u->dims[L - 1 - i];
        n += 3 * T(co, h, w);
        if (i < L - 1) { h *= 2; w *= 2; }
        n += T(ci, h, w);
    }
    n += T(u->dims[0], H, W);
    return n + 4096;
}

size_t scratch_bytes(const ofd_unet* u, int B, int H, int W) {
    const size_t px = (size_t)B * H * W;
    const int C = u->dims[0];
    size_t act = px * 2 * (size_t)(3 * C + C + 384 + 128 + C);
    size_t small = 4 * ofd_conv_gn_partial_count(B, H, W, u->dims[u->L]) * 4 + (size_t)B * 4 * ((size_t)(la_fwd_parts(B, H * W) > 256 ? la_fwd_parts(B, H * W) : 256) * 1088 + 1024) * 4 +
                   16 * (size_t)B * u->dims[u->L] * 4 + 64 * 1024;
    return act + small + 64 * 256;
}

size_t small_bytes(const ofd_unet* u, int B) {
    return ((size_t)B * u->ss_stride + 2 * (size_t)B * u->cfg.dim * 4) * 4 + 4096;
}

}

static void drop_graphs(ofd_unet* u);

static void upload_mlp_descs(ofd_unet* u) {
    if (u->cfg.no_time) return;
    std::vector<MlpDesc> descs;
    for (auto& name : u->resblocks) {
        MlpDesc d;
        d.weight = u->P(name + ".mlp.1.weight");
        d.bias = u->P(name + ".mlp.1.bias");
        d.n_out = (int)u->params[u->pindex.at(name + ".mlp.1.bias")].numel;
        d.offset = u->ss_offset.at(name);
        descs.push_back(d);
    }
    if (hipMemcpy(u->d_mlp, descs.data(), descs.size() * sizeof(MlpDesc), hipMemcpyHostToDevice) != hipSuccess)
        set_error("unet: uploading the time-projection descriptors failed");
}

extern "C" int ofd_unet_bind_param_buffer(ofd_unet* u, float* dev_params, size_t floats) {
    OFD_CHECK_ARG(u && dev_params, "unet_bind_param_buffer: null argument");
    OFD_CHECK_ARG(floats >= u->n_param_floats, "unet_bind_param_buffer: %zu floats, need %zu", floats, u->n_param_floats);
    OFD_CHECK_ARG(((uintptr_t)dev_params & 15) == 0, "unet_bind_param_buffer: buffer must be 16-byte aligned");
    if (u->owns_params && u->d_params) (void)hipFree(u->d_params);
    drop_graphs(u);
    if (u->d_prep) { (void)hipFree(u->d_prep); u->d_prep = nullptr; u->n_prep = 0; u->prep_blocks = 0; }
    u->d_params = dev_params;
    u->owns_params = false;
    for (auto& p : u->params) p.set = true;
    upload_mlp_descs(u);
    u->prepared = false;
    u->wt_prepared = false;
    return OFD_OK;
}

extern "C" int ofd_unet_create(const ofd_unet_config* cfg, ofd_unet** out) {
    OFD_CHECK_ARG(cfg && out, "unet_create: null argument");
    OFD_CHECK_ARG(cfg->dim == 64, "unet_create: dim=%d unsupported (the FlowDiffuser UNet is Unet(64), flow_diffuser.py:106)", cfg->dim);
    OFD_CHECK_ARG(cfg->channels >= 1 && cfg->channels <= 48, "unet_create: channels=%d (1..48)", cfg->channels);
    OFD_CHECK_ARG(cfg->out_dim >= 1 && cfg->out_dim <= 16, "unet_create: out_dim=%d (1..16)", cfg->out_dim);
    OFD_CHECK_ARG(cfg->n_levels == 0 || cfg->n_levels == 3 || cfg->n_levels == 4, "unet_create: n_levels=%d (0 or 4: dim_mults (1,2,4,8); 3: (1,2,4))",
                  cfg->n_levels);
    OFD_CHECK_ARG(cfg->n_levels != 3 || cfg->no_time == 1, "unet_create: the three-level UNet (the Autoencoder's) takes no time input (no_time=1)");
    OFD_CHECK_ARG(cfg->eps_mode == 0 || cfg->eps_mode == 1, "unet_create: eps_mode=%d", cfg->eps_mode);
    OFD_CHECK_ARG(cfg->no_time == 0 || cfg->no_time == 1, "unet_create: no_time=%d", cfg->no_time);
    ofd_unet* u = new ofd_unet();
    u->cfg = *cfg;
    u->L = cfg->n_levels == 3 ? 3 : 4;
    u->deterministic = env_int("OFD_DETERMINISTIC", 0) != 0;
    build_registry(u);
    if (hipMalloc(&u->d_params, u->n_param_floats * sizeof(float)) != hipSuccess ||
        hipMalloc(&u->d_wbuf, u->n_wbuf * sizeof(bf16_t)) != hipSuccess ||
        hipMalloc(&u->d_mlp, u->resblocks.size() * sizeof(MlpDesc)) != hipSuccess ||
        hipMalloc(&u->d_labuf, (u->n_labuf + 8) * sizeof(bf16_t)) != hipSuccess) {
        set_error("unet_create: hipMalloc failed");
        ofd_unet_destroy(u);
        return OFD_ERR_HIP;
    }
    if (hipMemset(u->d_params, 0, u->n_param_floats * sizeof(float)) != hipSuccess) {
        set_error("unet_create: hipMemset failed");
        ofd_unet_destroy(u);
        return OFD_ERR_HIP;
    }
    upload_mlp_descs(u);
    *out = u;
    return OFD_OK;
}

extern "C" void ofd_unet_destroy(ofd_unet* u) {
    if (!u) return;
    if (u->d_params && u->owns_params) (void)hipFree(u->d_params);
    if (u->d_wbuf) (void)hipFree(u->d_wbuf);
    if (u->d_mlp) (void)hipFree(u->d_mlp);
    if (u->d_labuf) (void)hipFree(u->d_labuf);
    if (u->d_wtbuf) (void)hipFree(u->d_wtbuf);
    if (u->d_wacc) (void)hipFree(u->d_wacc);
    if (u->d_fx) (void)hipFree(u->d_fx);
    if (u->d_det_miss) (void)hipFree(u->d_det_miss);
    if (u->d_prep) (void)hipFree(u->d_prep);
    if (u->d_tr) (void)hipFree(u->d_tr);
    drop_graphs(u);
    if (u->s2) {
        (void)hipStreamDestroy(u->s2);
        (void)hipEventDestroy(u->ev_fork); (void)hipEventDestroy(u->ev_join); (void)hipEventDestroy(u->ev_phase);
    }
    for (auto e : u->pool) (void)hipEventDestroy(e);
    delete u;
}

extern "C" int ofd_unet_num_params(const ofd_unet* u) { return u ? (int)u->params.size() : 0; }
extern "C" const char* ofd_unet_param_name(const ofd_unet* u, int i) {
    return (u && i >= 0 && i < (int)u->params.size()) ? u->params[i].name.c_str() : "";
}
extern "C" size_t ofd_unet_param_numel(const ofd_unet* u, int i) {
    return (u && i >= 0 && i < (int)u->params.size()) ? u->params[i].numel : 0;
}

extern "C" int ofd_unet_param_shape(const ofd_unet* u, int i, int* dims4) {
    if (!u || i < 0 || i >= (int)u->params.size() || !dims4) return 0;
    for (int k = 0; k < 4; ++k) dims4[k] = u->params[i].shape[k];
    return u->params[i].ndim;
}

extern "C" int ofd_unet_set_param(ofd_unet* u, int i, const float* dev_src, size_t numel, void* stream) {
    OFD_CHECK_ARG(u && dev_src && i >= 0 && i < (int)u->params.size(), "unet_set_param: bad argument");
    Param& p = u->params[i];
    OFD_CHECK_ARG(numel == p.numel, "unet_set_param: %s has %zu elements, got %zu", p.name.c_str(), p.numel, numel);
    OFD_HIP(hipMemcpyAsync(u->d_params + p.offset, dev_src, numel * sizeof(float), hipMemcpyDeviceToDevice, (hipStream_t)stream));
    p.set = true;
    u->prepared = false;
    u->wt_prepared = false;
    return OFD_OK;
}

extern "C" int ofd_unet_prepare(ofd_unet* u, void* stream) {
    OFD_CHECK_ARG(u, "unet_prepare: null handle");
    for (auto& p : u->params)
        if (!p.set) {
            set_error("unet_prepare: parameter %s was never set", p.name.c_str());
            return OFD_ERR_STATE;
        }
    if (!u->d_prep) {
        std::vector<ofd_weight_prep_desc> h;
        int blocks = 0;
        auto add = [&](const ConvDesc& c, size_t off, int cin_pad, int unshuffle) {
            ofd_weight_prep_desc d{u->P(c.wname), u->d_wbuf + off, c.Cout, c.Cin, cin_pad, c.ksize, c.ws_eps, unshuffle, blocks};
            h.push_back(d);
            blocks += c.Cout;
        };
        for (auto& c : u->convs) {
            add(c, c.w_off, c.Cin_pad, c.unshuffle);
            if (c.pack8_off >= 0) add(c, (size_t)c.pack8_off, 8, 0);
        }
        OFD_HIP(hipMalloc(&u->d_prep, h.size() * sizeof(ofd_weight_prep_desc)));
        OFD_HIP(hipMemcpy(u->d_prep, h.data(), h.size() * sizeof(ofd_weight_prep_desc), hipMemcpyHostToDevice));
        u->n_prep = (int)h.size();
        u->prep_blocks = blocks;
    }
    {
        int rc = k_conv_weight_prep_batched(u->d_prep, u->n_prep, u->prep_blocks, (hipStream_t)stream);
        if (rc != OFD_OK) return rc;
    }
    for (auto& c : u->convs) {
        if (c.phase_off >= 0) {
            int rc = ofd_conv_upsample_phase_weight_prep(u->P(c.wname), u->d_wbuf + c.phase_off, c.Cout, c.Cin, stream);
            if (rc != OFD_OK) return rc;
        }
    }
    for (auto& kv : u->la_fused) {
        const std::string& name = kv.first;
        const int C = kv.second.second;
        bf16_t* base = u->d_labuf + kv.second.first;
        int rc = k_la_weight_prep(u->P(name + ".fn.fn.to_qkv.weight"), u->P(name + ".fn.norm.g"), u->P(name + ".fn.fn.to_out.0.weight"),
                                  base, base + (size_t)128 * C, base + (size_t)384 * C, C, (hipStream_t)stream);
        if (rc != OFD_OK) return rc;
        if (C == 64) {
            rc = k_la_weight_prep(u->P(name + ".fn.fn.to_qkv.weight"), nullptr, nullptr, base + (size_t)512 * C, base + (size_t)640 * C, nullptr, C, (hipStream_t)stream);
            if (rc != OFD_OK) return rc;
        }
    }
    u->prepared = true;
    u->wt_prepared = false;
    return OFD_OK;
}

static size_t staging_bytes(const ofd_unet* u, int B, int H, int W) {
    auto al = [](size_t n) { return (n + 255) / 256 * 256; };
    return al((size_t)B * u->cfg.channels * H * W * 4) + al((size_t)B * 8) + al((size_t)B * u->cfg.out_dim * H * W * 4);
}

static size_t workspace_bytes_one(const ofd_unet* u, int B, int H, int W) {
    return persist_bytes(u, B, H, W) + scratch_bytes(u, B, H, W) + small_bytes(u, B) + 1024 + staging_bytes(u, B, H, W);
}

static size_t half_workspace_bytes(const ofd_unet* u, int B, int H, int W) { return (workspace_bytes_one(u, B / 2, H, W) + 255) / 256 * 256; }

extern "C" size_t ofd_unet_workspace_bytes(const ofd_unet* u, int B, int H, int W) {
    if (!u || B <= 0 || H <= 0 || W <= 0) return 0;
    const size_t one = workspace_bytes_one(u, B, H, W);
    if (B >= 2 && B % 2 == 0) { const size_t two = 2 * half_workspace_bytes(u, B, H, W); return two > one ? two : one; }
    return one;
}

static void drop_graphs(ofd_unet* u) {
    for (auto& g : u->graphs) {
        if (g.state == 2) { (void)hipGraphExecDestroy(g.exec); (void)hipGraphDestroy(g.graph); }
    }
    u->graphs.clear();
    if (u->cap_stream) { (void)hipStreamDestroy(u->cap_stream); u->cap_stream = nullptr; }
}

extern "C" int ofd_unet_set_graph(ofd_unet* u, int enabled) {
    OFD_CHECK_ARG(u, "unet_set_graph: null handle");
    u->graph_enabled = enabled != 0;
    if (!u->graph_enabled) drop_graphs(u);
    return OFD_OK;
}

extern "C" int ofd_unet_forward(ofd_unet* u, const float* x, int Cx, const float* cond, int Cc, const int64_t* t, float* out,
                                int B, int H, int W, void* workspace, size_t workspace_bytes, void* stream) {
    OFD_CHECK_ARG(u && x && (t || u->cfg.no_time) && out && workspace, "unet_forward: null argument");
    const int mult = 1 << (u->L - 1);
    OFD_CHECK_ARG(B > 0 && H > 0 && W > 0 && H % mult == 0 && W % mult == 0, "unet_forward: H=%d W=%d must be positive multiples of %d (%d 2x down-samplings, DD:95-99)",
                  H, W, mult, u->L - 1);
    OFD_CHECK_ARG(Cx + (cond ? Cc : 0) == u->cfg.channels, "unet_forward: %d + %d input channels, UNet has %d", Cx, cond ? Cc : 0, u->cfg.channels);
    if (!u->prepared) { set_error("unet_forward: call ofd_unet_prepare after setting parameters"); return OFD_ERR_STATE; }
    OFD_CHECK_WORKSPACE(workspace_bytes, ofd_unet_workspace_bytes(u, B, H, W), "unet_forward");
    OFD_CHECK_ARG(((uintptr_t)workspace & 255) == 0, "unet_forward: workspace must be 256-byte aligned");
    auto layout = [&](Ctx& c, int b, char* w_, size_t bytes, hipStream_t s_, float*& temb_, float*& temb_silu_) {
        c.u = u; c.s = s_; c.B = b;
        const size_t sb = (small_bytes(u, b) + 255) / 256 * 256;
        float* fsmall = (float*)w_;
        c.ss = fsmall;
        temb_ = fsmall + (size_t)b * u->ss_stride;
        temb_silu_ = temb_ + (size_t)b * u->cfg.dim * 4;
        c.persist = w_ + sb;
        c.persist_cap = persist_bytes(u, b, H, W);
        c.scratch = c.persist + (c.persist_cap + 255) / 256 * 256;
        c.scratch_cap = bytes - staging_bytes(u, b, H, W) - (size_t)(c.scratch - w_);
    };
    char* w = (char*)workspace;
    const bool split_auto = u->split_streams < 0 && (long)B * H * W >= (1L << 21);
    if ((u->split_streams > 0 || split_auto) && B >= 2 && B % 2 == 0 && !u->profiling && !u->graph_enabled) {
        if (!u->s2) {
            OFD_HIP(hipStreamCreateWithFlags(&u->s2, hipStreamNonBlocking));
            OFD_HIP(hipEventCreateWithFlags(&u->ev_fork, hipEventDisableTiming));
            OFD_HIP(hipEventCreateWithFlags(&u->ev_join, hipEventDisableTiming));
            OFD_HIP(hipEventCreateWithFlags(&u->ev_phase, hipEventDisableTiming));
        }
        const int hb = B / 2;
        const size_t hbytes = half_workspace_bytes(u, B, H, W);
        hipStream_t s1 = (hipStream_t)stream;
        Ctx c0, c1;
        float *te0, *ts0, *te1, *ts1;
        layout(c0, hb, w, hbytes, s1, te0, ts0);
        layout(c1, hb, w + hbytes, hbytes, u->s2, te1, ts1);
        const size_t plane = (size_t)H * W;
        c0.signal_at = u->split_offset; c0.signal_ev = u->ev_phase;
        OFD_HIP(hipEventRecord(u->ev_fork, s1));
        OFD_HIP(hipStreamWaitEvent(u->s2, u->ev_fork, 0));
        int rc = run_forward(c0, x, Cx, cond, Cc, t, out, H, W, te0, ts0), rc1 = OFD_OK;
        hipError_t he = hipSuccess;
        if (rc == OFD_OK) {
            if (!c0.signalled) he = hipEventRecord(u->ev_phase, s1);
            u->taps_half0 = u->taps;
            if (he == hipSuccess) he = hipStreamWaitEvent(u->s2, u->ev_phase, 0);
            if (he == hipSuccess)
                rc1 = run_forward(c1, x + (size_t)hb * Cx * plane, Cx, cond ? cond + (size_t)hb * Cc * plane : nullptr, Cc, t ? t + hb : nullptr,
                                  out + (size_t)hb * u->cfg.out_dim * plane, H, W, te1, ts1);
        }
        hipError_t hj = hipEventRecord(u->ev_join, u->s2);
        if (hj == hipSuccess) hj = hipStreamWaitEvent(s1, u->ev_join, 0);
        if (hj != hipSuccess) (void)hipStreamSynchronize(u->s2);
        if (he != hipSuccess || hj != hipSuccess) {
            set_error("unet_forward (split streams): %s", hipGetErrorString(he != hipSuccess ? he : hj));
            if (rc == OFD_OK && rc1 == OFD_OK) rc = OFD_ERR_HIP;
        }
        u->last_split = true;
        return rc != OFD_OK ? rc : rc1;
    }
    u->last_split = false;
    Ctx c;
    float *temb, *temb_silu;
    layout(c, B, w, workspace_bytes, (hipStream_t)stream, temb, temb_silu);
    const size_t stg = staging_bytes(u, B, H, W);
    if (!u->graph_enabled || u->profiling) return run_forward(c, x, Cx, cond, Cc, t, out, H, W, temb, temb_silu);

    auto al = [](size_t n) { return (n + 255) / 256 * 256; };
    char* sbase = w + workspace_bytes - stg;
    sbase = (char*)(((uintptr_t)sbase) & ~(uintptr_t)255);
    const size_t plane = (size_t)H * W * 4;
    float* sx = (float*)sbase;
    float* sc = sx + (size_t)B * Cx * H * W;
    int64_t* st = (int64_t*)(sbase + al((size_t)B * u->cfg.channels * plane));
    float* sout = (float*)((char*)st + al((size_t)B * 8));
    hipStream_t s_ = (hipStream_t)stream;
    OFD_HIP(hipMemcpyAsync(sx, x, (size_t)B * Cx * plane, hipMemcpyDeviceToDevice, s_));
    if (cond) OFD_HIP(hipMemcpyAsync(sc, cond, (size_t)B * Cc * plane, hipMemcpyDeviceToDevice, s_));
    if (t) OFD_HIP(hipMemcpyAsync(st, t, (size_t)B * 8, hipMemcpyDeviceToDevice, s_));
    ofd_unet::GraphEntry* e = nullptr;
    for (auto& g : u->graphs)
        if (g.workspace == workspace && g.B == B && g.H == H && g.W == W && g.Cx == Cx && g.Cc == (cond ? Cc : 0) && g.stream == s_) e = &g;
    int rc = OFD_OK;
    if (!e) {
        if (u->graphs.size() >= 8) drop_graphs(u);
        u->graphs.push_back({workspace, B, H, W, Cx, cond ? Cc : 0, s_, 0, nullptr, nullptr});
        rc = run_forward(c, sx, Cx, cond ? sc : nullptr, Cc, st, sout, H, W, temb, temb_silu);
    } else {
        if (e->state == 0) {
            if (!u->cap_stream) OFD_HIP(hipStreamCreateWithFlags(&u->cap_stream, hipStreamNonBlocking));
            OFD_HIP(hipStreamBeginCapture(u->cap_stream, hipStreamCaptureModeThreadLocal));
            c.s = u->cap_stream;
            rc = run_forward(c, sx, Cx, cond ? sc : nullptr, Cc, st, sout, H, W, temb, temb_silu);
            hipGraph_t g = nullptr;
            const hipError_t er = hipStreamEndCapture(u->cap_stream, &g);
            if (rc != OFD_OK || er != hipSuccess || !g) {
                if (g) (void)hipGraphDestroy(g);
                if (rc == OFD_OK) { set_error("unet_forward: stream capture failed: %s", hipGetErrorString(er)); rc = OFD_ERR_HIP; }
                return rc;
            }
            hipGraphExec_t ex = nullptr;
            OFD_HIP(hipGraphInstantiate(&ex, g, nullptr, nullptr, 0));
            e->graph = g; e->exec = ex; e->state = 2;
        }
        OFD_HIP(hipGraphLaunch(e->exec, s_));
    }
    if (rc != OFD_OK) return rc;
    OFD_HIP(hipMemcpyAsync(out, sout, (size_t)B * u->cfg.out_dim * plane, hipMemcpyDeviceToDevice, s_));
    return OFD_OK;
}

extern "C" int ofd_unet_set_split_streams(ofd_unet* u, int enabled, int offset_blocks) {
    OFD_CHECK_ARG(u, "unet_set_split_streams: null handle");
    u->split_streams = enabled < 0 ? -1 : (enabled != 0);
    if (offset_blocks >= 0) u->split_offset = offset_blocks;
    return OFD_OK;
}

extern "C" int ofd_unet_set_debug_taps(ofd_unet* u, int enabled) {
    OFD_CHECK_ARG(u, "unet_set_debug_taps: null handle");
    u->debug_taps = enabled != 0;
    return OFD_OK;
}

extern "C" int ofd_unet_set_glue(ofd_unet* u, int x_affine, int cond_affine, int out_mode, float out_div) {
    OFD_CHECK_ARG(u, "unet_set_glue: null handle");
    OFD_CHECK_ARG((x_affine == 0 || x_affine == 1) && (cond_affine == 0 || cond_affine == 1), "unet_set_glue: affine flags are 0 or 1");
    OFD_CHECK_ARG(out_mode >= 0 && out_mode <= 2, "unet_set_glue: out_mode=%d (0..2)", out_mode);
    OFD_CHECK_ARG(out_div > 0.0f, "unet_set_glue: out_div=%g must be positive", (double)out_div);
    u->glue_x = x_affine; u->glue_cond = cond_affine; u->glue_out = out_mode; u->glue_div = out_div;
    drop_graphs(u);
    return OFD_OK;
}

extern "C" int ofd_unet_read_tap(ofd_unet* u, const char* name, float* dst, size_t numel, void* stream) {
    OFD_CHECK_ARG(u && name && dst, "unet_read_tap: null argument");
    auto it = u->taps.find(name);
    OFD_CHECK_ARG(it != u->taps.end(), "unet_read_tap: no tap named '%s' in the last forward%s", name,
                  std::string(name) == "final_res_block" ? " (that tensor is only materialised after ofd_unet_set_debug_taps(u, 1): the final 1x1 conv normally rides on its producer)" : "");
    const Tensor& t = it->second;
    const int halves = u->last_split ? 2 : 1;
    OFD_CHECK_ARG(numel == (size_t)halves * u->last_B * t.C * t.H * t.W, "unet_read_tap: %s has %zu elements, got %zu", name,
                  (size_t)halves * u->last_B * t.C * t.H * t.W, numel);
    if (u->last_split) {
        const Tensor& t0 = u->taps_half0.at(name);
        int rc = k_nhwc_to_nchw(t0.p, dst, u->last_B, t.H, t.W, t.C, (hipStream_t)stream);
        if (rc != OFD_OK) return rc;
        dst += (size_t)u->last_B * t.C * t.H * t.W;
    }
    return k_nhwc_to_nchw(t.p, dst, u->last_B, t.H, t.W, t.C, (hipStream_t)stream);
}

extern "C" int ofd_unet_set_profiling(ofd_unet* u, int enabled) {
    OFD_CHECK_ARG(u, "unet_set_profiling: null handle");
    u->profiling = enabled != 0;
    return OFD_OK;
}
extern "C" int ofd_unet_prof_dump_path(ofd_unet* u, const char* path) {
    OFD_CHECK_ARG(u, "unet_prof_dump_path: null handle");
    u->dump_path = path ? path : "";
    return OFD_OK;
}
namespace ofd {
const char* prof_class_name(int cls) {
    static std::string names[PC_COUNT];
    static bool built = false;
    if (!built) {
        const std::string c64 = env_int("OFD_CONV_PC", 1) ? "conv3x3_pc_kernel" : "conv3x3_wp_kernel<2,2>";
        names[PC_CONV3] = "conv3x3_wp16_kernel [3x3, Cout a multiple of 128]";
        names[PC_CONV3_64] = c64 + " [3x3, Cin > 64 -> 64]";
        names[PC_CONV3_PP] = c64 + " [3x3, 64 -> 64]";
        names[PC_CONV1] = "conv1x1_wp_kernel | conv_igemm_kernel<1,BN> [1x1]";
        names[PC_CONV7] = std::string(env_int("OFD_CONV7_PERSIST", 1) ? "conv7x7_c8_persist_kernel" : "conv_igemm_kernel<8,64>") + " [7x7 init conv]";
        names[PC_GN] = "gn_finalize";
        names[PC_RESOUT] = "resblock_out";
        names[PC_LN] = "layernorm_c";
        names[PC_LINATTN] = "la_ctx_fused + la_out_fused | lc_* [LinearAttention]";
        names[PC_FLASH] = "flash_attn_d32 [mid attention]";
        names[PC_MISC] = "misc";
        names[PC_WGRAD3] = "conv_wgrad3 [3x3 weight gradients]";
        names[PC_WGRAD1] = "conv_wgrad1 [1x1 / 7x7 weight gradients]";
        names[PC_DGRAD3] = "conv3x3 data gradients [forward kernels on dY]";
        names[PC_DGRAD1] = "conv1x1 data gradients";
        names[PC_GNBWD] = "gn_silu_backward";
        names[PC_LABWD] = "linear_attention_backward";
        names[PC_FLASHBWD] = "flash_attention_backward";
        names[PC_CONVUP] = "conv_up2_phases_wp_kernel [Upsample x2 + 3x3 as four 2x2 phase convs]";
        names[PC_DGRAD7] = "conv7_dgrad_kernel [7x7 init conv data gradient]";
        built = true;
    }
    return (cls >= 0 && cls < PC_COUNT) ? names[cls].c_str() : "";
}
}

extern "C" int ofd_unet_prof_count(const ofd_unet* u) { return u ? PC_COUNT : 0; }
extern "C" const char* ofd_unet_prof_name(const ofd_unet* u, int i) { return (u && i >= 0 && i < PC_COUNT) ? prof_class_name(i) : ""; }

static int prof_resolve(ofd_unet* u) {
    FILE* dump = u->dump_path.empty() ? nullptr : fopen(u->dump_path.c_str(), "a");
    for (auto& r : u->recs) {
        OFD_HIP(hipEventSynchronize(r.e1));
        float ms = 0.0f;
        OFD_HIP(hipEventElapsedTime(&ms, r.e0, r.e1));
        if (dump) fprintf(dump, "%s,%s,%.4f,%.6g,%.6g\n", prof_class_name(r.cls), r.label.c_str(), ms, r.flops, r.bytes);
        u->acc_ms[r.cls] += ms;
        u->acc_flops[r.cls] += r.flops;
        u->acc_bytes[r.cls] += r.bytes;
        u->acc_launch[r.cls] += 1;
    }
    if (dump) fclose(dump);
    u->recs.clear();
    u->pool_used = 0;
    return OFD_OK;
}

extern "C" int ofd_unet_prof_read(ofd_unet* u, int i, double* ms, long long* launches, double* flops, double* bytes) {
    OFD_CHECK_ARG(u && i >= 0 && i < PC_COUNT, "unet_prof_read: bad argument");
    int rc = prof_resolve(u);
    if (rc != OFD_OK) return rc;
    if (ms) *ms = u->acc_ms[i];
    if (launches) *launches = u->acc_launch[i];
    if (flops) *flops = u->acc_flops[i];
    if (bytes) *bytes = u->acc_bytes[i];
    return OFD_OK;
}

extern "C" int ofd_unet_prof_reset(ofd_unet* u) {
    OFD_CHECK_ARG(u, "unet_prof_reset: null handle");
    int rc = prof_resolve(u);
    for (int i = 0; i < PC_COUNT; ++i) { u->acc_ms[i] = 0; u->acc_flops[i] = 0; u->acc_bytes[i] = 0; u->acc_launch[i] = 0; }
    return rc;
}
```

Measured before the change: 35.30.

## Extend fused linear-attention block to 256 and 512 channel levels

Extends the fused linear-attention inference path, previously limited to C≤128, to C=256 and C=512, so the deeper UNet levels no longer take the unfused multi-kernel path. For C=512 the context kernel splits the four heads across two blocks (grid z) so the weights fit in LDS. The output stage is split into a heads kernel and a tail kernel, with y used as the intermediate buffer. Occupancy drops to one block per CU at these widths, the grid sizing changes, and an env var can disable the wide path.

```diff
diff --git a/opticalflowdiffusion_amd/csrc/attn_bwd.hip b/opticalflowdiffusion_amd/csrc/attn_bwd.hip
--- a/opticalflowdiffusion_amd/csrc/attn_bwd.hip
+++ b/opticalflowdiffusion_amd/csrc/attn_bwd.hip
@@ -235,14 +235,14 @@
 static inline bool al16(const void* p) { return ((uintptr_t)p & 15) == 0; }
 extern "C" int ofd_la_weight_prep(const float* wqkv, const float* g, const float* wout, void* wq, void* wkv, void* woutp, int C, void* stream) {
     OFD_CHECK_ARG(wqkv && wq && wkv && (woutp == nullptr) == (wout == nullptr), "la_weight_prep: null argument (wout and woutp go together)");
-    OFD_CHECK_ARG(C == 64 || C == 128, "la_weight_prep: C=%d (64 or 128)", C);
+    OFD_CHECK_ARG(C == 64 || C == 128 || C == 256 || C == 512, "la_weight_prep: C=%d (64, 128, 256 or 512)", C);
     OFD_CHECK_ARG(al16(wq) && al16(wkv) && al16(woutp), "la_weight_prep: weight buffers must be 16-byte aligned");
     return k_la_weight_prep(wqkv, g, wout, (bf16_t*)wq, (bf16_t*)wkv, (bf16_t*)woutp, C, (hipStream_t)stream);
 }
 extern "C" int ofd_linear_attention_block(const void* x, const void* wq, const void* wkv, const void* woutp, const float* bias, const float* g2,
                                           float* partial, void* ctxfrag, void* y, int B, int n, int C, float eps_pre, float eps_post, void* stream) {
     OFD_CHECK_ARG(x && wq && wkv && woutp && bias && g2 && partial && ctxfrag && y, "linear_attention_block: null argument");
-    OFD_CHECK_ARG(C == 64 || C == 128, "linear_attention_block: C=%d (64 or 128)", C);
+    OFD_CHECK_ARG(C == 64 || C == 128 || C == 256 || C == 512, "linear_attention_block: C=%d (64, 128, 256 or 512)", C);
     OFD_CHECK_ARG(B > 0 && n > 0, "linear_attention_block: B=%d n=%d", B, n);
     OFD_CHECK_ARG(al16(x) && al16(y) && al16(wq) && al16(wkv) && al16(woutp) && al16(ctxfrag), "linear_attention_block: x, y, ctxfrag and the weights must be 16-byte aligned");
     return k_linear_attention_fused((const bf16_t*)x, (const bf16_t*)wq, (const bf16_t*)wkv, (const bf16_t*)woutp, bias, g2, partial, (bf16_t*)ctxfrag,
diff --git a/opticalflowdiffusion_amd/csrc/blocks.h b/opticalflowdiffusion_amd/csrc/blocks.h
--- a/opticalflowdiffusion_amd/csrc/blocks.h
+++ b/opticalflowdiffusion_amd/csrc/blocks.h
@@ -45,7 +45,7 @@
 int la_parts(int B, int n);
 int k_linear_attention_core(const bf16_t* qkv, float* partial, float* ctx, bf16_t* out, int B, int n, hipStream_t s, float* ml_out = nullptr,
                             const bf16_t* wo = nullptr, const float* bo = nullptr, bf16_t* o2 = nullptr, int C = 0);
-int la_fused_blocks(int n, int B);
+int la_fused_blocks(int n, int B, int C = 64);
 int la_fwd_parts(int B, int n);
 int k_linear_attention_fused_train(const bf16_t* x, const bf16_t* wq, const bf16_t* wkv, const bf16_t* woutp, const float* bias, const float* g_pre,
                                    const float* g2, float* partial, bf16_t* ctxfrag, float* ctx, float* ml, bf16_t* xn, bf16_t* qkv, bf16_t* o2,
diff --git a/opticalflowdiffusion_amd/csrc/la_fused.hip b/opticalflowdiffusion_amd/csrc/la_fused.hip
--- a/opticalflowdiffusion_amd/csrc/la_fused.hip
+++ b/opticalflowdiffusion_amd/csrc/la_fused.hip
@@ -14,6 +14,22 @@
 __device__ __forceinline__ void load_raw_x(const bf16_t* __restrict__ xrow, XRaw<C>& r, int half) {
 #pragma unroll
     for (int s = 0; s < C / 16; ++s) r.v[s] = *(const u32x4*)(xrow + 16 * s + 8 * half);
+}
+
+template <int N16, class At>
+__device__ __forceinline__ void la_stage(unsigned char* dst, const bf16_t* __restrict__ src, int tid, At at) {
+    static_assert(N16 % (8 * 256) == 0, "whole turns of eight units per thread");
+    for (int i0 = tid; i0 < N16; i0 += 8 * 256) {
+        uint4 v[8];
+#pragma unroll
+        for (int k = 0; k < 8; ++k) v[k] = ((const uint4*)src)[at(i0 + k * 256)];
+#pragma unroll
+        for (int k = 0; k < 8; ++k) ((uint4*)dst)[i0 + k * 256] = v[k];
+    }
+}
+template <int N16>
+__device__ __forceinline__ void la_stage(unsigned char* dst, const bf16_t* __restrict__ src, int tid) {
+    la_stage<N16>(dst, src, tid, [](int i) { return i; });
 }
 
 typedef __bf16 la_bf16x2 __attribute__((ext_vector_type(2)));
@@ -107,9 +123,10 @@
     __syncthreads();
 }
 
-__device__ __forceinline__ void ctx_state_init(f32x16 (&ctxT)[4], float (&m)[4], float (&l)[4]) {
-#pragma unroll
-    for (int hd = 0; hd < 4; ++hd) {
+template <int NH>
+__device__ __forceinline__ void ctx_state_init(f32x16 (&ctxT)[NH], float (&m)[NH], float (&l)[NH]) {
+#pragma unroll
+    for (int hd = 0; hd < NH; ++hd) {
         m[hd] = -3.0e38f;
         l[hd] = 0.0f;
 #pragma unroll
@@ -135,23 +152,32 @@
     for (int s2 = 0; s2 < 2; ++s2) ctxT = __builtin_amdgcn_mfma_f32_32x32x16_bf16(acc_frag(va, s2), acc_frag(p, s2), ctxT, 0, 0, 0);
 }
 
-template <int C, bool TRAIN>
-__global__ void __launch_bounds__(256, 2) la_ctx_fused_kernel(const bf16_t* __restrict__ x, const bf16_t* __restrict__ wkv,
+template <int C, bool TRAIN, int HPW = 4>
+__global__ void __launch_bounds__(256, C >= 256 ? 1 : 2) la_ctx_fused_kernel(const bf16_t* __restrict__ x, const bf16_t* __restrict__ wkv,
                                                            float* __restrict__ partial, int n, float eps, float defer,
                                                            const float* __restrict__ g, bf16_t* __restrict__ xn_out, bf16_t* __restrict__ qkv_out) {
     extern __shared__ __attribute__((aligned(16))) unsigned char smem[];
-    constexpr int KS = C / 16;
+    static_assert(HPW == 4 || (HPW == 2 && !TRAIN), "the training form writes all four heads' k | v");
+    constexpr int KS = C / 16, WR = 64 * HPW;
     const int tid = threadIdx.x, lane = tid & 63, wave = tid >> 6, l31 = lane & 31, half = lane >> 5;
-    for (int i = tid; i < (C / 8) * 256; i += 256) ((uint4*)smem)[i] = ((const uint4*)wkv)[i];
-    float* s_g = (float*)(smem + (C / 8) * 256 * 16);
+    const int h0 = HPW == 4 ? 0 : blockIdx.z * HPW;
+    if constexpr (C < 256) {
+        for (int i = tid; i < (C / 8) * 256; i += 256) ((uint4*)smem)[i] = ((const uint4*)wkv)[i];
+    } else {
+        la_stage<(C / 8) * WR>(smem, wkv, tid, [&](int i) {
+            const int r = i % WR, kv = r / (32 * HPW);
+            return (i / WR) * 256 + kv * 128 + h0 * 32 + (r - kv * 32 * HPW);
+        });
+    }
+    float* s_g = (float*)(smem + (C / 8) * WR * 16);
     if constexpr (TRAIN)
         for (int i = tid; i < C; i += 256) s_g[i] = g[i];
     __syncthreads();
     const int b = blockIdx.y, wave_id = blockIdx.x * 4 + wave, nw = gridDim.x * 4, ntiles = (n + 31) / 32;
 
-    f32x16 ctxT[4];
-    float m[4], l[4];
-    ctx_state_init(ctxT, m, l);
+    f32x16 ctxT[HPW];
+    float m[HPW], l[HPW];
+    ctx_state_init<HPW>(ctxT, m, l);
     const bf16_t* xb = x + (size_t)b * n * C;
     XRaw<C> raw_next;
     load_raw_x<C>(xb + (size_t)min(wave_id * 32 + l31, n - 1) * C, raw_next, half);
@@ -185,14 +211,14 @@
             }
         }
 #pragma unroll
-        for (int hd = 0; hd < 4; ++hd) {
+        for (int hd = 0; hd < HPW; ++hd) {
             f32x16 ka, va;
 #pragma unroll
             for (int r = 0; r < 16; ++r) { ka[r] = 0.0f; va[r] = 0.0f; }
 #pragma unroll
             for (int s = 0; s < KS; ++s) {
-                const bf16x8 wk = *(const bf16x8*)(smem + ((size_t)(2 * s + half) * 256 + hd * 32 + l31) * 16);
-                const bf16x8 wv = *(const bf16x8*)(smem + ((size_t)(2 * s + half) * 256 + 128 + hd * 32 + l31) * 16);
+                const bf16x8 wk = *(const bf16x8*)(smem + ((size_t)(2 * s + half) * WR + hd * 32 + l31) * 16);
+                const bf16x8 wv = *(const bf16x8*)(smem + ((size_t)(2 * s + half) * WR + 32 * HPW + hd * 32 + l31) * 16);
                 ka = __builtin_amdgcn_mfma_f32_32x32x16_bf16(xs[s], wk, ka, 0, 0, 0);
                 va = __builtin_amdgcn_mfma_f32_32x32x16_bf16(xs[s], wv, va, 0, 0, 0);
             }
@@ -230,8 +256,8 @@
     }
     __syncthreads();
 #pragma unroll
-    for (int hd = 0; hd < 4; ++hd)
-        la_store_part((float*)smem, partial + ((size_t)(b * 4 + hd) * gridDim.x + blockIdx.x) * 1088, m[hd], l[hd], ctxT[hd], tid, wave, l31, half);
+    for (int hd = 0; hd < HPW; ++hd)
+        la_store_part((float*)smem, partial + ((size_t)(b * 4 + h0 + hd) * gridDim.x + blockIdx.x) * 1088, m[hd], l[hd], ctxT[hd], tid, wave, l31, half);
 }
 
 __global__ void __launch_bounds__(256, 2) la_ctx_stored_kernel(const bf16_t* __restrict__ qkv, float* __restrict__ partial, int n) {
@@ -390,7 +416,98 @@
 }
 
 template <int C, bool TRAIN>
-__global__ void __launch_bounds__(256, C == 64 ? 4 : 2) la_out_fused_kernel(const bf16_t* __restrict__ x, const bf16_t* __restrict__ wq,
+__device__ __forceinline__ f32x16 la_head_out(const bf16x8 (&xs)[C / 16], const unsigned char* s_wq, const unsigned char* s_cf, int hd, float scale,
+                                              int lane) {
+    const int l31 = lane & 31, half = lane >> 5;
+    f32x16 qa;
+#pragma unroll
+    for (int r = 0; r < 16; ++r) qa[r] = 0.0f;
+#pragma unroll
+    for (int s = 0; s < C / 16; ++s) {
+        const bf16x8 wf = *(const bf16x8*)(s_wq + ((size_t)(2 * s + half) * 128 + hd * 32 + l31) * 16);
+        qa = __builtin_amdgcn_mfma_f32_32x32x16_bf16(wf, xs[s], qa, 0, 0, 0);
+    }
+    if constexpr (TRAIN) {
+#pragma unroll
+        for (int r = 0; r < 16; ++r) qa[r] = bf2f(f2bf(qa[r]));
+    }
+    const float k = scale / softmax_d(qa, 32);
+#pragma unroll
+    for (int r = 0; r < 16; ++r) qa[r] *= k;
+    f32x16 oa;
+#pragma unroll
+    for (int r = 0; r < 16; ++r) oa[r] = 0.0f;
+#pragma unroll
+    for (int s2 = 0; s2 < 2; ++s2) {
+        const bf16x8 cf = *(const bf16x8*)(s_cf + ((size_t)(hd * 2 + s2) * 64 + lane) * 16);
+        oa = __builtin_amdgcn_mfma_f32_32x32x16_bf16(cf, acc_frag(qa, s2), oa, 0, 0, 0);
+    }
+    return oa;
+}
+template <int C>
+__device__ __forceinline__ void la_to_out(f32x16 (&acc_o)[C / 32], const bf16x8 of, const unsigned char* s_wo, int u, int l31, int half) {
+#pragma unroll
+    for (int rt = 0; rt < C / 32; ++rt) {
+        const bf16x8 wf = *(const bf16x8*)(s_wo + ((size_t)(u * 2 + half) * C + rt * 32 + l31) * 16);
+        acc_o[rt] = __builtin_amdgcn_mfma_f32_32x32x16_bf16(wf, of, acc_o[rt], 0, 0, 0);
+    }
+}
+template <int C, bool TRAIN, class XRes>
+__device__ __forceinline__ void la_out_tail(f32x16 (&acc_o)[C / 32], XRes xres, const float* s_bias, const float* s_g2, bf16_t* yrow, bf16_t* orow, bool ok,
+                                            int half, float eps_post) {
+    constexpr int RT = C / 32;
+    float sum = 0.0f;
+#pragma unroll
+    for (int rt = 0; rt < RT; ++rt)
+#pragma unroll
+        for (int g = 0; g < 4; ++g) {
+            const float4 bv = *(const float4*)(s_bias + rt * 32 + 8 * g + 4 * half);
+            acc_o[rt][4 * g] += bv.x; acc_o[rt][4 * g + 1] += bv.y; acc_o[rt][4 * g + 2] += bv.z; acc_o[rt][4 * g + 3] += bv.w;
+            if constexpr (TRAIN) {
+#pragma unroll
+                for (int k = 0; k < 4; ++k) acc_o[rt][4 * g + k] = bf2f(f2bf(acc_o[rt][4 * g + k]));
+            }
+            sum += (acc_o[rt][4 * g] + acc_o[rt][4 * g + 1]) + (acc_o[rt][4 * g + 2] + acc_o[rt][4 * g + 3]);
+        }
+    if constexpr (TRAIN) {
+#pragma unroll
+        for (int rt = 0; rt < RT; ++rt) store_acc_rows(acc_o[rt], orow + rt * 32, half, ok);
+    }
+    sum += __shfl_xor(sum, 32, 64);
+    const float mean = sum * (1.0f / C);
+    float q = 0.0f;
+#pragma unroll
+    for (int rt = 0; rt < RT; ++rt)
+#pragma unroll
+        for (int r = 0; r < 16; ++r) { acc_o[rt][r] -= mean; q += acc_o[rt][r] * acc_o[rt][r]; }
+    q += __shfl_xor(q, 32, 64);
+    const float rstd = rsqrtf(q * (1.0f / C) + eps_post);
+#pragma unroll
+    for (int rt = 0; rt < RT; ++rt)
+#pragma unroll
+        for (int g = 0; g < 4; g += 2) {
+            const u32x4 xw = xres(rt * 2 + (g >> 1));
+            const uint4 xv = make_uint4(xw[0], xw[1], xw[2], xw[3]);
+            const auto sx = __builtin_amdgcn_permlane32_swap(xv.x, xv.z, false, false);
+            const auto sy = __builtin_amdgcn_permlane32_swap(xv.y, xv.w, false, false);
+            const unsigned xq[2][2] = {{sx[0], sy[0]}, {sx[1], sy[1]}};
+            uint2 qo[2];
+#pragma unroll
+            for (int k = 0; k < 2; ++k) {
+                const int c0 = rt * 32 + 8 * (g + k) + 4 * half;
+                const float4 gv = *(const float4*)(s_g2 + c0);
+                const float o0 = acc_o[rt][4 * (g + k)] * rstd * gv.x + bf2f((bf16_t)(xq[k][0] & 0xffffu));
+                const float o1 = acc_o[rt][4 * (g + k) + 1] * rstd * gv.y + bf2f((bf16_t)(xq[k][0] >> 16));
+                const float o2 = acc_o[rt][4 * (g + k) + 2] * rstd * gv.z + bf2f((bf16_t)(xq[k][1] & 0xffffu));
+                const float o3 = acc_o[rt][4 * (g + k) + 3] * rstd * gv.w + bf2f((bf16_t)(xq[k][1] >> 16));
+                qo[k] = pack_quad(o0, o1, o2, o3);
+            }
+            store_quad_pair(yrow + rt * 32 + 8 * g, qo[0], qo[1], half, ok);
+        }
+}
+
+template <int C, bool TRAIN>
+__global__ void __launch_bounds__(256, C == 64 ? 4 : C == 128 ? 2 : 1) la_out_fused_kernel(const bf16_t* __restrict__ x, const bf16_t* __restrict__ wq,
                                                            const bf16_t* __restrict__ woutp, const bf16_t* __restrict__ ctxfrag,
                                                            const float* __restrict__ bias, const float* __restrict__ g2,
                                                            bf16_t* __restrict__ y, int n, float eps_pre, float eps_post, float scale,
@@ -408,8 +525,13 @@
     const int b = blockIdx.y;
     if constexpr (TRAIN)
         for (int i = tid; i < C; i += 256) s_g[i] = g[i];
-    for (int i = tid; i < WQ_B / 16; i += 256) ((uint4*)s_wq)[i] = ((const uint4*)wq)[i];
-    for (int i = tid; i < WO_B / 16; i += 256) ((uint4*)s_wo)[i] = ((const uint4*)woutp)[i];
+    if constexpr (C < 256) {
+        for (int i = tid; i < WQ_B / 16; i += 256) ((uint4*)s_wq)[i] = ((const uint4*)wq)[i];
+        for (int i = tid; i < WO_B / 16; i += 256) ((uint4*)s_wo)[i] = ((const uint4*)woutp)[i];
+    } else {
+        la_stage<WQ_B / 16>(s_wq, wq, tid);
+        la_stage<WO_B / 16>(s_wo, woutp, tid);
+    }
     for (int i = tid; i < CF_B / 16; i += 256) ((uint4*)s_cf)[i] = ((const uint4*)(ctxfrag + (size_t)b * 4096))[i];
     for (int i = tid; i < C; i += 256) { s_bias[i] = bias[i]; s_g2[i] = g2[i]; }
     __syncthreads();
@@ -421,8 +543,7 @@
     for (int tile = wave_id; tile < ntiles; tile += nw) {
         asm volatile("" ::: "memory");
         const int pix = tile * 32 + l31;
-        const int pid = min(pix, n - 1);
-        const bf16_t* xrow = xb + (size_t)pid * C;
+        const size_t row = (size_t)b * n + min(pix, n - 1);
         const XRaw<C> raw = raw_next;
         load_raw_x<C>(xb + (size_t)min((tile + nw) * 32 + l31, n - 1) * C, raw_next, half);
         bf16x8 xs[KS];
@@ -435,92 +556,91 @@
             for (int r = 0; r < 16; ++r) acc_o[rt][r] = 0.0f;
 #pragma unroll
         for (int hd = 0; hd < 4; ++hd) {
-            f32x16 qa;
-#pragma unroll
-            for (int r = 0; r < 16; ++r) qa[r] = 0.0f;
-#pragma unroll
-            for (int s = 0; s < KS; ++s) {
-                const bf16x8 wf = *(const bf16x8*)(s_wq + ((size_t)(2 * s + half) * 128 + hd * 32 + l31) * 16);
-                qa = __builtin_amdgcn_mfma_f32_32x32x16_bf16(wf, xs[s], qa, 0, 0, 0);
-            }
-            if constexpr (TRAIN) {
-#pragma unroll
-                for (int r = 0; r < 16; ++r) qa[r] = bf2f(f2bf(qa[r]));
-            }
-            const float k = scale / softmax_d(qa, 32);
-#pragma unroll
-            for (int r = 0; r < 16; ++r) qa[r] *= k;
-            f32x16 oa;
-#pragma unroll
-            for (int r = 0; r < 16; ++r) oa[r] = 0.0f;
-#pragma unroll
-            for (int s2 = 0; s2 < 2; ++s2) {
-                const bf16x8 cf = *(const bf16x8*)(s_cf + ((size_t)(hd * 2 + s2) * 64 + lane) * 16);
-                oa = __builtin_amdgcn_mfma_f32_32x32x16_bf16(cf, acc_frag(qa, s2), oa, 0, 0, 0);
-            }
-#pragma unroll
-            for (int s2 = 0; s2 < 2; ++s2) {
-                const bf16x8 of = acc_frag(oa, s2);
-#pragma unroll
-                for (int rt = 0; rt < RT; ++rt) {
-                    const bf16x8 wf = *(const bf16x8*)(s_wo + ((size_t)((hd * 2 + s2) * 2 + half) * C + rt * 32 + l31) * 16);
-                    acc_o[rt] = __builtin_amdgcn_mfma_f32_32x32x16_bf16(wf, of, acc_o[rt], 0, 0, 0);
-                }
-            }
-        }
-        float sum = 0.0f;
+            const f32x16 oa = la_head_out<C, TRAIN>(xs, s_wq, s_cf, hd, scale, lane);
+#pragma unroll
+            for (int s2 = 0; s2 < 2; ++s2) la_to_out<C>(acc_o, acc_frag(oa, s2), s_wo, hd * 2 + s2, l31, half);
+        }
+        la_out_tail<C, TRAIN>(acc_o, [&](int s) { return raw.v[s]; }, s_bias, s_g2, y + row * C, TRAIN ? o2_out + row * C : nullptr, pix < n, half, eps_post);
+    }
+}
+
+template <int C>
+__global__ void __launch_bounds__(256, 1) la_heads_kernel(const bf16_t* __restrict__ x, const bf16_t* __restrict__ wq, const bf16_t* __restrict__ ctxfrag,
+                                                          bf16_t* __restrict__ y, int n, float eps_pre, float scale) {
+    extern __shared__ __attribute__((aligned(16))) unsigned char smem[];
+    constexpr int WQ_B = (C / 8) * 128 * 16, CF_B = 4 * 2 * 64 * 16;
+    unsigned char* s_wq = smem;
+    unsigned char* s_cf = smem + WQ_B;
+    const int tid = threadIdx.x, lane = tid & 63, wave = tid >> 6, l31 = lane & 31, half = lane >> 5;
+    const int b = blockIdx.y;
+    la_stage<WQ_B / 16>(s_wq, wq, tid);
+    for (int i = tid; i < CF_B / 16; i += 256) ((uint4*)s_cf)[i] = ((const uint4*)(ctxfrag + (size_t)b * 4096))[i];
+    __syncthreads();
+    const int wave_id = blockIdx.x * 4 + wave, nw = gridDim.x * 4, ntiles = (n + 31) / 32;
+    const bf16_t* xb = x + (size_t)b * n * C;
+    XRaw<C> raw_next;
+    load_raw_x<C>(xb + (size_t)min(wave_id * 32 + l31, n - 1) * C, raw_next, half);
+    for (int tile = wave_id; tile < ntiles; tile += nw) {
+        asm volatile("" ::: "memory");
+        const int pix = tile * 32 + l31;
+        const XRaw<C> raw = raw_next;
+        load_raw_x<C>(xb + (size_t)min((tile + nw) * 32 + l31, n - 1) * C, raw_next, half);
+        bf16x8 xs[C / 16];
+        norm_x<C>(raw, eps_pre, xs);
+        bf16_t* arow = y + ((size_t)b * n + min(pix, n - 1)) * C + 8 * half;
+#pragma unroll
+        for (int hd = 0; hd < 4; ++hd) {
+            const f32x16 oa = la_head_out<C, false>(xs, s_wq, s_cf, hd, scale, lane);
+#pragma unroll
+            for (int s2 = 0; s2 < 2; ++s2)
+                if (pix < n) *(bf16x8*)(arow + (hd * 2 + s2) * 16) = acc_frag(oa, s2);
+        }
+    }
+}
+
+template <int C>
+__global__ void __launch_bounds__(256, 1) la_tail_kernel(const bf16_t* __restrict__ x, const bf16_t* __restrict__ woutp, const float* __restrict__ bias,
+                                                         const float* __restrict__ g2, bf16_t* y, int n, float eps_post) {
+    extern __shared__ __attribute__((aligned(16))) unsigned char smem[];
+    constexpr int RT = C / 32, WO_B = 16 * C * 16;
+    unsigned char* s_wo = smem;
+    float* s_bias = (float*)(smem + WO_B);
+    float* s_g2 = s_bias + C;
+    const int tid = threadIdx.x, lane = tid & 63, wave = tid >> 6, l31 = lane & 31, half = lane >> 5;
+    const int b = blockIdx.y;
+    la_stage<WO_B / 16>(s_wo, woutp, tid);
+    for (int i = tid; i < C; i += 256) { s_bias[i] = bias[i]; s_g2[i] = g2[i]; }
+    __syncthreads();
+    const int wave_id = blockIdx.x * 4 + wave, nw = gridDim.x * 4, ntiles = (n + 31) / 32;
+    const bf16_t* xb = x + (size_t)b * n * C;
+    bf16_t* yb = y + (size_t)b * n * C;
+    bf16x8 of_next[8];
+    {
+        const bf16_t* arow = yb + (size_t)min(wave_id * 32 + l31, n - 1) * C + 8 * half;
+#pragma unroll
+        for (int u = 0; u < 8; ++u) of_next[u] = *(const bf16x8*)(arow + u * 16);
+    }
+    for (int tile = wave_id; tile < ntiles; tile += nw) {
+        asm volatile("" ::: "memory");
+        const int pix = tile * 32 + l31;
+        const size_t pid = min(pix, n - 1);
+        bf16x8 of[8];
+#pragma unroll
+        for (int u = 0; u < 8; ++u) of[u] = of_next[u];
+        {
+            const bf16_t* arow = yb + (size_t)min((tile + nw) * 32 + l31, n - 1) * C + 8 * half;
+#pragma unroll
+            for (int u = 0; u < 8; ++u) of_next[u] = *(const bf16x8*)(arow + u * 16);
+        }
+        f32x16 acc_o[RT];
 #pragma unroll
         for (int rt = 0; rt < RT; ++rt)
 #pragma unroll
-            for (int g = 0; g < 4; ++g) {
-                const float4 bv = *(const float4*)(s_bias + rt * 32 + 8 * g + 4 * half);
-                acc_o[rt][4 * g] += bv.x; acc_o[rt][4 * g + 1] += bv.y; acc_o[rt][4 * g + 2] += bv.z; acc_o[rt][4 * g + 3] += bv.w;
-                if constexpr (TRAIN) {
-#pragma unroll
-                    for (int k = 0; k < 4; ++k) acc_o[rt][4 * g + k] = bf2f(f2bf(acc_o[rt][4 * g + k]));
-                }
-                sum += (acc_o[rt][4 * g] + acc_o[rt][4 * g + 1]) + (acc_o[rt][4 * g + 2] + acc_o[rt][4 * g + 3]);
-            }
-        if constexpr (TRAIN) {
-            bf16_t* orow = o2_out + ((size_t)b * n + min(pix, n - 1)) * C;
-#pragma unroll
-            for (int rt = 0; rt < RT; ++rt) store_acc_rows(acc_o[rt], orow + rt * 32, half, pix < n);
-        }
-        sum += __shfl_xor(sum, 32, 64);
-        const float mean = sum * (1.0f / C);
-        float q = 0.0f;
-#pragma unroll
-        for (int rt = 0; rt < RT; ++rt)
-#pragma unroll
-            for (int r = 0; r < 16; ++r) { acc_o[rt][r] -= mean; q += acc_o[rt][r] * acc_o[rt][r]; }
-        q += __shfl_xor(q, 32, 64);
-        const float rstd = rsqrtf(q * (1.0f / C) + eps_post);
-        {
-            const bool ok = pix < n;
-            bf16_t* yrow = y + ((size_t)b * n + min(pix, n - 1)) * C;
-#pragma unroll
-            for (int rt = 0; rt < RT; ++rt)
-#pragma unroll
-                for (int g = 0; g < 4; g += 2) {
-                    const u32x4 xw = raw.v[rt * 2 + (g >> 1)];
-                    const uint4 xv = make_uint4(xw[0], xw[1], xw[2], xw[3]);
-                    const auto sx = __builtin_amdgcn_permlane32_swap(xv.x, xv.z, false, false);
-                    const auto sy = __builtin_amdgcn_permlane32_swap(xv.y, xv.w, false, false);
-                    const unsigned xq[2][2] = {{sx[0], sy[0]}, {sx[1], sy[1]}};
-                    uint2 qo[2];
-#pragma unroll
-                    for (int k = 0; k < 2; ++k) {
-                        const int c0 = rt * 32 + 8 * (g + k) + 4 * half;
-                        const float4 gv = *(const float4*)(s_g2 + c0);
-                        const float o0 = acc_o[rt][4 * (g + k)] * rstd * gv.x + bf2f((bf16_t)(xq[k][0] & 0xffffu));
-                        const float o1 = acc_o[rt][4 * (g + k) + 1] * rstd * gv.y + bf2f((bf16_t)(xq[k][0] >> 16));
-                        const float o2 = acc_o[rt][4 * (g + k) + 2] * rstd * gv.z + bf2f((bf16_t)(xq[k][1] & 0xffffu));
-                        const float o3 = acc_o[rt][4 * (g + k) + 3] * rstd * gv.w + bf2f((bf16_t)(xq[k][1] >> 16));
-                        qo[k] = pack_quad(o0, o1, o2, o3);
-                    }
-                    store_quad_pair(yrow + rt * 32 + 8 * g, qo[0], qo[1], half, ok);
-                }
-        }
+            for (int r = 0; r < 16; ++r) acc_o[rt][r] = 0.0f;
+#pragma unroll
+        for (int u = 0; u < 8; ++u) la_to_out<C>(acc_o, of[u], s_wo, u, l31, half);
+        const bf16_t* xrow = xb + pid * C + 8 * half;
+        la_out_tail<C, false>(acc_o, [&](int s) { return *(const u32x4*)(xrow + 16 * s); }, s_bias, s_g2, yb + pid * C, nullptr, pix < n, half, eps_post);
     }
 }
 
@@ -546,7 +666,11 @@
 
 constexpr float LA_DEFER = 5.545177f;
 constexpr int LA_GX2_CAP = 128;
-static int la_out_blocks(int n, int B) {
+static int la_out_blocks(int n, int B, int C) {
+    if (C >= 256) {
+        const int gx2 = cdiv(cdiv(n, 32), 4), cap2 = 256 / B;
+        return gx2 < cap2 ? gx2 : (cap2 < 1 ? 1 : cap2);
+    }
     int gx2 = cdiv(cdiv(n, 32), 4 * 4);
     if (gx2 < 1) gx2 = 1;
     const int cap2 = (LA_GX2_CAP * B < 1024) ? 1024 / B : LA_GX2_CAP;
@@ -557,18 +681,32 @@
 template <int C>
 static int launch_la(const bf16_t* x, const bf16_t* wq, const bf16_t* wkv, const bf16_t* woutp, const float* bias, const float* g2,
                      float* partial, bf16_t* ctxfrag, bf16_t* y, int B, int n, float eps_pre, float eps_post, hipStream_t s) {
-    constexpr int LDS1 = (C / 8) * 256 * 16;
+    constexpr int HPW = C == 512 ? 2 : 4;
+    constexpr bool SPLIT2 = C == 512;
+    constexpr int LDS1 = (C / 8) * 64 * HPW * 16;
     constexpr int LDS2 = (C / 8) * 128 * 16 + 16 * C * 16 + 4 * 2 * 64 * 16 + 2 * C * 4;
+    constexpr int LDS2H = (C / 8) * 128 * 16 + 4 * 2 * 64 * 16, LDS2T = 16 * C * 16 + 2 * C * 4;
+    static_assert(LDS1 <= 160 * 1024 && (SPLIT2 ? LDS2H <= 160 * 1024 && LDS2T <= 160 * 1024 : LDS2 <= 160 * 1024), "the weights of a pass must fit the LDS");
     static bool attr = false;
     if (!attr) {
-        OFD_HIP(hipFuncSetAttribute((const void*)la_ctx_fused_kernel<C, false>, hipFuncAttributeMaxDynamicSharedMemorySize, LDS1));
-        OFD_HIP(hipFuncSetAttribute((const void*)la_out_fused_kernel<C, false>, hipFuncAttributeMaxDynamicSharedMemorySize, LDS2));
+        OFD_HIP(hipFuncSetAttribute((const void*)la_ctx_fused_kernel<C, false, HPW>, hipFuncAttributeMaxDynamicSharedMemorySize, LDS1));
+        if constexpr (SPLIT2) {
+            OFD_HIP(hipFuncSetAttribute((const void*)la_heads_kernel<C>, hipFuncAttributeMaxDynamicSharedMemorySize, LDS2H));
+            OFD_HIP(hipFuncSetAttribute((const void*)la_tail_kernel<C>, hipFuncAttributeMaxDynamicSharedMemorySize, LDS2T));
+        } else {
+            OFD_HIP(hipFuncSetAttribute((const void*)la_out_fused_kernel<C, false>, hipFuncAttributeMaxDynamicSharedMemorySize, LDS2));
+        }
         attr = true;
     }
-    const int gx = la_fused_blocks(n, B);
-    la_ctx_fused_kernel<C, false><<<dim3(gx, B), 256, LDS1, s>>>(x, wkv, partial, n, eps_pre, LA_DEFER, nullptr, nullptr, nullptr);
+    const int gx = la_fused_blocks(n, B, C), gx2 = la_out_blocks(n, B, C);
+    la_ctx_fused_kernel<C, false, HPW><<<dim3(gx, B, 4 / HPW), 256, LDS1, s>>>(x, wkv, partial, n, eps_pre, LA_DEFER, nullptr, nullptr, nullptr);
     la_ctx_combine_kernel<<<dim3(B * 4, 4), 256, 0, s>>>(partial, ctxfrag, gx, 1.0f / (float)n, nullptr);
-    la_out_fused_kernel<C, false><<<dim3(la_out_blocks(n, B), B), 256, LDS2, s>>>(x, wq, woutp, ctxfrag, bias, g2, y, n, eps_pre, eps_post, LA_SCALE, nullptr, nullptr);
+    if constexpr (SPLIT2) {
+        la_heads_kernel<C><<<dim3(gx2, B), 256, LDS2H, s>>>(x, wq, ctxfrag, y, n, eps_pre, LA_SCALE);
+        la_tail_kernel<C><<<dim3(gx2, B), 256, LDS2T, s>>>(x, woutp, bias, g2, y, n, eps_post);
+    } else {
+        la_out_fused_kernel<C, false><<<dim3(gx2, B), 256, LDS2, s>>>(x, wq, woutp, ctxfrag, bias, g2, y, n, eps_pre, eps_post, LA_SCALE, nullptr, nullptr);
+    }
     OFD_LAUNCH_CHECK();
     return OFD_OK;
 }
@@ -589,16 +727,18 @@
     la_ctx_fused_kernel<64, true><<<dim3(gx, B), 256, LDS1, s>>>(x, wkv, partial, n, eps_pre, LA_DEFER, g_pre, xn, qkv);
     la_ctx_combine_kernel<<<dim3(B * 4, 4), 256, 0, s>>>(partial, ctxfrag, gx, 1.0f / (float)n, nullptr);
     launch_la_ctx_combine(partial, ctx, B, gx, 1.0f / (float)n, ml, s);
-    la_out_fused_kernel<64, true><<<dim3(la_out_blocks(n, B), B), 256, LDS2, s>>>(x, wq, woutp, ctxfrag, bias, g2, y, n, eps_pre, eps_post, LA_SCALE, g_pre, o2);
+    la_out_fused_kernel<64, true><<<dim3(la_out_blocks(n, B, 64), B), 256, LDS2, s>>>(x, wq, woutp, ctxfrag, bias, g2, y, n, eps_pre, eps_post, LA_SCALE, g_pre, o2);
     OFD_LAUNCH_CHECK();
     return OFD_OK;
 }
 
-int la_fused_blocks(int n, int B) {
+int la_fused_blocks(int n, int B, int C) {
     constexpr int total = 256;
     int gx = cdiv(cdiv(n, 32), 8);
     int cap = total / (B < 1 ? 1 : B);
-    if (cap < 64) cap = 64;
+    if (C >= 256) cap = (cap < 32 ? 32 : cap) / (C / 256);
+    else if (cap < 64) cap = 64;
+    if (cap < 1) cap = 1;
     if (gx < 1) gx = 1;
     if (gx > cap) gx = cap;
     return gx;
@@ -614,6 +754,8 @@
                              float* partial, bf16_t* ctxfrag, bf16_t* y, int B, int n, int C, float eps_pre, float eps_post, hipStream_t s) {
     if (C == 64) return launch_la<64>(x, wq, wkv, woutp, bias, g2, partial, ctxfrag, y, B, n, eps_pre, eps_post, s);
     if (C == 128) return launch_la<128>(x, wq, wkv, woutp, bias, g2, partial, ctxfrag, y, B, n, eps_pre, eps_post, s);
+    if (C == 256) return launch_la<256>(x, wq, wkv, woutp, bias, g2, partial, ctxfrag, y, B, n, eps_pre, eps_post, s);
+    if (C == 512) return launch_la<512>(x, wq, wkv, woutp, bias, g2, partial, ctxfrag, y, B, n, eps_pre, eps_post, s);
     set_error("linear_attention_fused: C=%d unsupported", C);
     return OFD_ERR_ARG;
 }
diff --git a/opticalflowdiffusion_amd/csrc/unet.hip b/opticalflowdiffusion_amd/csrc/unet.hip
--- a/opticalflowdiffusion_amd/csrc/unet.hip
+++ b/opticalflowdiffusion_amd/csrc/unet.hip
@@ -59,11 +59,9 @@
     add_conv(u, name + ".fn.fn.to_out.0", c, 128, 1, true, -1.0f);
     add_param(u, name + ".fn.fn.to_out.1.g", {1, c, 1, 1});
     add_param(u, name + ".fn.norm.g", {1, c, 1, 1});
-    if (c <= 128) {
-        u->la_fused[name] = {u->n_labuf, c};
-        u->n_labuf += (size_t)512 * c;
-        if (c == 64) u->n_labuf += (size_t)384 * c;
-    }
+    u->la_fused[name] = {u->n_labuf, c};
+    u->n_labuf += (size_t)512 * c;
+    if (c == 64) u->n_labuf += (size_t)384 * c;
 }
 
 static void build_registry(ofd_unet* u) {
@@ -212,8 +210,8 @@
     const int H = x.H, W = x.W, B = c.B, C = x.C, n = H * W;
     const size_t npix = (size_t)B * n;
     auto fit = u->la_fused.find(name);
-    if (fit != u->la_fused.end() && !c.train) {
-        const int nparts = la_fused_blocks(n, B);
+    if (fit != u->la_fused.end() && !c.train && (C <= 128 || env_int("OFD_LA_FUSED_WIDE", 1))) {
+        const int nparts = la_fused_blocks(n, B, C);
         float* partial = c.tmpf((size_t)B * 4 * nparts * 1088);
         bf16_t* ctxfrag = (bf16_t*)c.tmpf((size_t)B * 2048);
         Tensor y = c.keep(C, H, W);
```

New measurement: 35.70 (median of 6 runs). 1.1% higher.
